# google/ghost-dataplane

Measured on AMD Instinct MI355X. Metric: Mpkt/s device-resident coprocessor NF pipeline (64B pkts); HBM GB/s vs peak, higher is better.
Workload: dtype u32

## Files before the change

### ghost-dataplane_amd/csrc/cop_device.h

```cpp
#ifndef COP_DEVICE_H
#define COP_DEVICE_H

#include <hip/hip_runtime.h>
#include <stdint.h>

#include "cop_kernels.h"

namespace copd {

constexpr int BLOCK = COPK_BLOCK;
constexpr int WAVES = BLOCK / 64;

typedef uint32_t u32x2 __attribute__((ext_vector_type(2)));
typedef uint32_t u32x4 __attribute__((ext_vector_type(4)));
typedef uint32_t u32x4a __attribute__((ext_vector_type(4), aligned(4)));
typedef uint32_t u32x2a __attribute__((ext_vector_type(2), aligned(4)));

__device__ __forceinline__ uint32_t bswap32(uint32_t x) { return __builtin_bswap32(x); }

__device__ __forceinline__ void lb_store(unsigned long long *p, unsigned long long v)
{
    __hip_atomic_store(p, v, __ATOMIC_RELAXED, __HIP_MEMORY_SCOPE_AGENT);
}

// ... 66 lines not shown
__device__ __forceinline__ void lds_stage(uint32_t *lds_dst, const void *gsrc, uint32_t n16, int lane, int wave)
{
    const uint4 *g = (const uint4 *)gsrc;
    for (uint32_t c = (uint32_t)wave; c * 64u < n16; c += WAVES) {
        const uint32_t i = c * 64u + (uint32_t)lane;
        if (i < n16)
            __builtin_amdgcn_global_load_lds((const __attribute__((address_space(1))) void *)(g + i),
                                             (__attribute__((address_space(3))) void *)(lds_dst + c * 256u),
                                             16, 0, 0);
    }
}

__device__ __forceinline__ uint32_t ivt_search(const uint32_t *S, uint32_t m, uint32_t ib, uint32_t lv, uint32_t ip)
{
    const uint16_t *idx = (const uint16_t *)(S + m);
    const uint32_t b = ip >> (32u - ib);
    uint32_t k = idx[b];
    const uint32_t hi = idx[b + 1];
    for (uint32_t step = (1u << lv) >> 1; step; step >>= 1) {
        const uint32_t c = min(k + step, hi);
        if (S[c] <= ip) k = c;
    }
    return k;
}

#ifndef COPK_IVT_VALUE
#define COPK_IVT_VALUE 1
#endif
__device__ __forceinline__ uint32_t ivt_value(const uint32_t *S, const uint32_t *V, uint32_t m, uint32_t ib, uint32_t lv,
                                              uint32_t ip)
{
    if (!COPK_IVT_VALUE || lv == 0) return V[ivt_search(S, m, ib, lv, ip)];
    const uint16_t *idx = (const uint16_t *)(S + m);
    const uint32_t b = ip >> (32u - ib);
    uint32_t k = idx[b];
    const uint32_t hi = idx[b + 1];
    for (uint32_t step = (1u << lv) >> 1; step > 1; step >>= 1) {
        const uint32_t c = min(k + step, hi);
        if (S[c] <= ip) k = c;
    }
    const uint32_t c = min(k + 1, hi);
    const uint32_t sc = S[c], vk = V[k], vc = V[c];
    return sc <= ip ? vc : vk;
}

constexpr int LB_GROUPS = 4;
constexpr uint32_t LB_GAVE_UP = 0xFFFFFFFFu;
__device__ __forceinline__ uint32_t look_back(unsigned long long *chain, uint32_t stride, uint32_t j, uint32_t agg,
                                              uint32_t epoch, uint32_t *err, int lane, const uint32_t *exitw = nullptr,
                                              uint32_t spin_log2 = 22)
{
    const unsigned long long ep = (unsigned long long)epoch << 32;
    if (j == 0) {
        if (lane == 0) lb_store(&chain[0], ep | (2ull << 30) | agg);
        return 0;
    }
    if (lane == 0) lb_store(&chain[(size_t)j * stride], ep | (1ull << 30) | agg);
    uint32_t excl = 0;
    int qhi = (int)j - 1;
    uint32_t spins = 0;
    for (;;) {
        unsigned long long v[LB_GROUPS];
#pragma unroll
        for (int r = 0; r < LB_GROUPS; r++) {
            const int idx = qhi - r * 64 - lane;
            v[r] = idx >= 0 ? lb_load(&chain[(size_t)idx * stride]) : 0ull;
        }
        int consumed = 0;
        bool done = false;
#pragma unroll
        for (int r = 0; r < LB_GROUPS; r++) {
            const bool inb = qhi - r * 64 - lane >= 0;
            const uint32_t flag = (uint32_t)(v[r] >> 30) & 3u;
            const bool ok = inb && (uint32_t)(v[r] >> 32) == epoch && flag != 0u;
            const unsigned long long m_incl = __ballot(ok && flag == 2u);
            const unsigned long long m_bad = __ballot(inb && !ok);
            const int first_incl = m_incl ? __ffsll((long long)m_incl) - 1 : 64;
            const int first_bad = m_bad ? __ffsll((long long)m_bad) - 1 : 64;
            const int upto = min(first_incl + 1, first_bad);
            uint32_t val = lane < upto ? ((uint32_t)v[r] & 0x3FFFFFFFu) : 0u;
#pragma unroll
            for (int off = 32; off; off >>= 1) val += __shfl_xor(val, off);
            excl += val;
            consumed += upto;
            if (first_incl < first_bad) {
                done = true;
                break;
            }
            if (upto < 64) break;
        }
        if (done) break;
        qhi -= consumed;
        if (consumed == 0) {
            if (++spins > (1u << spin_log2)) {
                if (lane == 0) *err = 1u;
                if (exitw) return LB_GAVE_UP;
                break;
            }
            if (exitw && (spins & 63u) == 0 &&
                __hip_atomic_load(exitw, __ATOMIC_RELAXED, __HIP_MEMORY_SCOPE_AGENT) == COPK_PMD_ABORT)
                return LB_GAVE_UP;
            __builtin_amdgcn_s_sleep(1);
        }
    }
    if (lane == 0) lb_store(&chain[(size_t)j * stride], ep | (2ull << 30) | (excl + agg));
    return excl;
}

__device__ __forceinline__ uint32_t look_back_seg(unsigned long long *chain, uint32_t K, uint32_t gi, uint32_t agg,
                                                  uint32_t epoch, uint32_t *err, int lane)
{
    const uint32_t seg = K == 1 ? 64u : K == 2 ? 32u : K <= 4 ? 16u : 8u;
    const uint32_t q = (uint32_t)lane / seg, r = (uint32_t)lane % seg;
    const bool active = q < K;
    const unsigned long long segm = seg == 64 ? ~0ull : ((1ull << seg) - 1ull) << (q * seg);
    const uint32_t sh = seg == 64 ? 0u : q * seg;
    const unsigned long long ep = (unsigned long long)epoch << 32;
    uint32_t excl = 0;
    int qhi = (int)gi - 1;
    bool done = !active || gi == 0;
    uint32_t spins = 0;
    while (__ballot(!done)) {
        const int idx = qhi - (int)r;
        const bool inb = !done && idx >= 0;
        const unsigned long long v = inb ? lb_load(&chain[(size_t)idx * K + q]) : 0ull;
        const uint32_t flag = (uint32_t)(v >> 30) & 3u;
        const bool ok = inb && (uint32_t)(v >> 32) == epoch && flag != 0u;
        const unsigned long long mi = (__ballot(ok && flag == 2u) & segm) >> sh;
        const unsigned long long mb = (__ballot(inb && !ok) & segm) >> sh;
        const uint32_t first_incl = mi ? (uint32_t)__ffsll((long long)mi) - 1u : seg;
        const uint32_t first_bad = mb ? (uint32_t)__ffsll((long long)mb) - 1u : seg;
        const uint32_t upto = min(first_incl + 1u, first_bad);
        uint32_t val = (inb && r < upto) ? ((uint32_t)v & 0x3FFFFFFFu) : 0u;
        for (uint32_t off = seg >> 1; off; off >>= 1) val += __shfl_xor(val, (int)off);
        bool stalled = false;
        if (!done) {
            excl += val;
            if (first_incl < first_bad) {
                done = true;
            } else {
                qhi -= (int)upto;
                stalled = upto == 0;
            }
        }
        if (__ballot(stalled)) {
            if (++spins > (1u << 22)) {
                if (lane == 0) *err = 1u;
                break;
            }
            __builtin_amdgcn_s_sleep(1);
        }
    }
    if (active && r == 0 && gi != 0) lb_store(&chain[(size_t)gi * K + q], ep | (2ull << 30) | (excl + agg));
    return excl;
}

__device__ __forceinline__ void lb_publish(unsigned long long *chain, uint32_t K, uint32_t gi, uint32_t agg_q,
                                           uint32_t epoch, int lane)
{
    if ((uint32_t)lane < K)
        lb_store(&chain[(size_t)gi * K + (uint32_t)lane],
                 ((unsigned long long)epoch << 32) | ((gi == 0 ? 2ull : 1ull) << 30) | agg_q);
}

__device__ __forceinline__ uint32_t wave_excl_scan(uint32_t c, int n, int lane, uint32_t *agg)
{
    uint32_t inc = c;
#pragma unroll
    for (int off = 1; off < 64; off <<= 1) {
        const uint32_t u = __shfl_up(inc, off);
        if (lane >= off) inc += u;
    }
    *agg = __shfl(inc, n - 1);
    return inc - c;
}

__device__ __forceinline__ CopKBatch batch_desc(const CopKParams &p, uint32_t b, uint32_t *look_off)
{
    CopKBatch B;
    if (p.ring) {
        const uint32_t slot = (p.rg.first + b) % p.rg.n_slots;
        B.pkts = p.rg.pkts + (size_t)slot * p.rg.pkts_slot_bytes;
        B.offsets = p.rg.offsets ? p.rg.offsets + (size_t)slot * p.rg.offsets_slot_words : nullptr;
        B.results = (uint2 *)p.rg.results + (size_t)slot * p.rg.results_slot;
        B.fwd_idx = p.rg.fwd_idx ? p.rg.fwd_idx + (size_t)slot * p.rg.fwd_slot : nullptr;
        const uint32_t per = p.seg ? (p.rg.n + COPK_SEG - 1u) / COPK_SEG : p.demux ? p.demux : 1u;
        B.fwd_count = p.rg.fwd_count ? p.rg.fwd_count + (size_t)slot * per : nullptr;
        B.n = p.rg.n;
        B.stride = p.rg.stride;
        B.data_off = p.rg.data_off;
        B.ntiles = p.uniform_ntiles;
        *look_off = b * p.uniform_ntiles;
    } else {
        B = p.b[b];
        *look_off = p.look_begin[b];
    }
    return B;
}

__device__ __forceinline__ uint32_t batch_of_tile(const CopKParams &p, uint32_t g)
{
    uint32_t b = 0;
    if (p.uniform_ntiles) {
        b = g / p.uniform_ntiles;
    } else {
#pragma unroll
        for (int q = 1; q < COPK_MAXB; q++) b += (q < (int)p.nb && p.tile_begin[q] <= g) ? 1u : 0u;
    }
    return __builtin_amdgcn_readfirstlane(b);
}

struct StepGeom {
    uint32_t lpk[3], lch[3];
    uint32_t r3;
    int a3, a67, a8;
};

__device__ __forceinline__ StepGeom step_geom(int lane)
{
    StepGeom g;
#pragma unroll
    for (int c = 0; c < 3; c++) {
        const uint32_t q = (uint32_t)(c * 64 + lane);
        g.lpk[c] = q / 3u;
        g.lch[c] = (q % 3u) * 16u;
    }
    g.r3 = (uint32_t)lane % 3u;
    g.a3 = ((3 * lane) & 63) << 2;
    g.a67 = ((3 * lane + 1) & 63) << 2;
    g.a8 = ((3 * lane + 2) & 63) << 2;
    return g;
}

__device__ __forceinline__ __amdgpu_buffer_rsrc_t sys_rsrc(const void *base)
{
    return __builtin_amdgcn_make_buffer_rsrc((void *)base, 0, 0x7FFFFFFF, 0x00020000);
}
__device__ __forceinline__ u32x4 ld_sys16(__amdgpu_buffer_rsrc_t rs, uint32_t off)
{
    return __builtin_amdgcn_raw_buffer_load_b128(rs, (int)off, 0, 1 | 16);
}
__device__ __forceinline__ u32x2 ld_sys8(__amdgpu_buffer_rsrc_t rs, uint32_t off)
{
    return __builtin_amdgcn_raw_buffer_load_b64(rs, (int)off, 0, 1 | 16);
}
__device__ __forceinline__ uint32_t ld_sys4(__amdgpu_buffer_rsrc_t rs, uint32_t off)
{
    return __builtin_amdgcn_raw_buffer_load_b32(rs, (int)off, 0, 1 | 16);
}

__device__ __forceinline__ void load_step(const StepGeom &g, const uint8_t *pk0, uint32_t stride, uint32_t pb,
                                          uint32_t last, u32x4 (&v)[3], bool sys = false)
{
    if (sys) {
        const __amdgpu_buffer_rsrc_t rs = sys_rsrc(pk0);
#pragma unroll
        for (int c = 0; c < 3; c++) v[c] = ld_sys16(rs, min(pb + g.lpk[c], last) * stride + g.lch[c]);
        return;
    }
#pragma unroll
    for (int c = 0; c < 3; c++) {
        const uint32_t ic = min(pb + g.lpk[c], last);
        v[c] = __builtin_nontemporal_load((const u32x4 *)(pk0 + (size_t)ic * stride + g.lch[c]));
    }
}

__device__ __forceinline__ void load_step_imix(const StepGeom &g, const uint8_t *pkts, uint32_t off,
                                               uint32_t data_off, u32x4 (&v)[3], bool sys = false)
{
    uint32_t o[3];
#pragma unroll
    for (int c = 0; c < 3; c++)
        o[c] = (uint32_t)__builtin_amdgcn_ds_bpermute((int)(g.lpk[c] << 2), (int)off) + data_off + g.lch[c];
    if (sys) {
        const __amdgpu_buffer_rsrc_t rs = sys_rsrc(pkts);
#pragma unroll
        for (int c = 0; c < 3; c++) v[c] = ld_sys16(rs, o[c]);
        return;
    }
#pragma unroll
    for (int c = 0; c < 3; c++) v[c] = __builtin_nontemporal_load((const u32x4 *)(pkts + o[c]));
}

__device__ __forceinline__ uint32_t load_off_imix(const uint32_t *offsets, uint32_t pb, int lane, uint32_t last,
                                                  bool sys = false)
{
    const uint32_t ic = min(pb + (uint32_t)lane, last);
    return sys ? ld_sys4(sys_rsrc(offsets), ic * 4u) : offsets[ic];
}

__device__ __forceinline__ void gather_step(const StepGeom &g, const u32x4 (&v)[3], uint32_t &w3, uint32_t &w6,
                                            uint32_t &w7, uint32_t &w8)
{
    const uint32_t c0w = g.r3 == 0 ? v[0].w : g.r3 == 1 ? v[2].w : v[1].w;
    const uint32_t c1z = g.r3 == 0 ? v[1].z : g.r3 == 1 ? v[0].z : v[2].z;
    const uint32_t c1w = g.r3 == 0 ? v[1].w : g.r3 == 1 ? v[0].w : v[2].w;
    const uint32_t c2x = g.r3 == 0 ? v[2].x : g.r3 == 1 ? v[1].x : v[0].x;
    w3 = (uint32_t)__builtin_amdgcn_ds_bpermute(g.a3, (int)c0w);
    w6 = (uint32_t)__builtin_amdgcn_ds_bpermute(g.a67, (int)c1z);
    w7 = (uint32_t)__builtin_amdgcn_ds_bpermute(g.a67, (int)c1w);
    w8 = (uint32_t)__builtin_amdgcn_ds_bpermute(g.a8, (int)c2x);
}

struct Opt {
    uint32_t demux;
    uint32_t port_stats;
    uint32_t dbg;
    unsigned long long *rule_hits;
};

__device__ __forceinline__ Opt opt_all(const CopKParams &p)
{
    return Opt{p.demux, p.port_stats, p.dbg, p.rule_hits};
}

struct Tables {
    uint32_t *rt_top;
    uint16_t *rt_leaf;
    uint32_t *fw_s, *fw_v, *lp_s, *lp_v;
};

__device__ __forceinline__ uint32_t probe_ld(const uint32_t *a, uint32_t nt)
{
    return nt ? __builtin_nontemporal_load(a) : *a;
}

__device__ __forceinline__ void bkt_issue(const uint32_t *bidx, uint32_t ib, uint32_t ip, bool reach, uint32_t &k0,
                                          uint32_t &k1)
{
    if (reach) {
        const u32x2a x = *(const u32x2a *)(bidx + (ip >> (32u - ib)));
        k0 = x.x;
        k1 = x.y;
    } else {
        k0 = k1 = 0;
    }
}

template <int FW, int LPM, int PPT>
__device__ __forceinline__ void pass1(const CopKParams &p, const Tables &t, const uint32_t (&w3)[PPT],
                                      const uint32_t (&w6)[PPT], const uint32_t (&w7)[PPT],
                                      const uint32_t (&w8)[PPT], uint32_t (&verdict)[PPT], uint32_t (&port)[PPT],
                                      uint32_t (&src)[PPT], uint32_t (&dst)[PPT], uint32_t (&fwe)[PPT],
                                      uint32_t (&lpe)[PPT], uint32_t (&lpe2)[PPT], uint32_t (&fwe2)[PPT])
{
    const bool stageP = (p.stages & COPK_STAGE_PARSE) != 0;
#pragma unroll
    for (int k = 0; k < PPT; k++) {
        verdict[k] = COPK_FORWARD;
        port[k] = 0;
        const uint32_t et = ((w3[k] & 0xFFu) << 8) | ((w3[k] >> 8) & 0xFFu);
        dst[k] = bswap32(__builtin_amdgcn_alignbit(w8[k], w7[k], 16));
        src[k] = bswap32(__builtin_amdgcn_alignbit(w7[k], w6[k], 16));
        if (stageP) {
            if (et != 0x0800u) {
                verdict[k] = COPK_DROP_PARSE;
                port[k] = 0xFFFFu;
            } else {
                const uint32_t idx = dst[k] & 0xFFFFu;
                const uint32_t top = t.rt_top[idx >> 8];
                port[k] = (top & 0x80000000u) ? (uint32_t)t.rt_leaf[((top & 0xFFFFu) << 8) | (idx & 0xFFu)]
                                              : (top & 0xFFFFu);
                if (port[k] == 0xFFFFu) verdict[k] = COPK_DROP_PARSE;
                else if (port[k] >= p.n_ports) verdict[k] = COPK_DROP_NO_PORT;
            }
        }
        const bool reach = verdict[k] == COPK_FORWARD;
        if (FW == COPK_TBL_IVT) fwe[k] = ivt_value(t.fw_s, t.fw_v, p.fw_m, p.fw_ib, p.fw_lv, src[k]);
        if (FW == COPK_TBL_DIR) fwe[k] = reach ? probe_ld(&p.fw_tbl24[src[k] >> 8], p.probe_nt) : 0u;
        if (FW == COPK_TBL_BKT) bkt_issue(p.fw_bidx, p.fw_ib, src[k], reach, fwe[k], fwe2[k]);
        if (LPM == COPK_TBL_IVT) lpe[k] = ivt_value(t.lp_s, t.lp_v, p.lpm_m, p.lpm_ib, p.lpm_lv, dst[k]);
        if (LPM == COPK_TBL_DIR) lpe[k] = reach ? probe_ld(&p.lpm_tbl24[dst[k] >> 8], p.probe_nt) : 0u;
        if (LPM == COPK_TBL_TRIE) lpe[k] = t.lp_s[dst[k] >> 20];
        if (LPM == COPK_TBL_BKT) bkt_issue(p.lpm_bidx, p.lpm_ib, dst[k], reach, lpe[k], lpe2[k]);
    }
}

template <int PPT>
__device__ __forceinline__ void trie_walk(const uint32_t *nodes, const uint32_t *leaves, const uint32_t (&ip)[PPT],
                                          uint32_t (&e)[PPT], const bool (&live)[PPT])
{
    bool in[PPT], lf[PPT];
    bool any = false;
#pragma unroll
    for (int k = 0; k < PPT; k++) {
        in[k] = live[k] && (e[k] & 0x80000000u);
        lf[k] = false;
        any |= in[k];
    }
#pragma unroll
    for (int l = 0; l < 4; l++) {
        if (!__ballot(any)) break;
        const uint32_t sh = l == 0 ? 14u : l == 1 ? 8u : l == 2 ? 2u : 0u;
        const uint32_t msk = l == 3 ? 3u : 63u;
        u32x4a a[PPT];
        u32x2a b[PPT];
#pragma unroll
        for (int k = 0; k < PPT; k++) {
            if (in[k]) {
                const uint32_t *nd = nodes + (size_t)(e[k] & 0x7FFFFFFFu) * 6u;
                a[k] = *(const u32x4a *)nd;
                b[k] = *(const u32x2a *)(nd + 4);
            }
        }
        any = false;
#pragma unroll
        for (int k = 0; k < PPT; k++) {
            if (in[k]) {
                const uint32_t c = (ip[k] >> sh) & msk;
                const unsigned long long vec = a[k].x | ((unsigned long long)a[k].y << 32);
                const unsigned long long lv = a[k].z | ((unsigned long long)a[k].w << 32);
                const unsigned long long upto = (2ull << c) - 1ull;
                if ((vec >> c) & 1ull) {
                    e[k] = 0x80000000u | (b[k].x + (uint32_t)__popcll(vec & upto) - 1u);
                    any = true;
                } else {
                    e[k] = b[k].y + (uint32_t)__popcll(lv & upto) - 1u;
                    in[k] = false;
                    lf[k] = true;
                }
            }
        }
    }
#pragma unroll
    for (int k = 0; k < PPT; k++)
        if (lf[k]) e[k] = leaves[e[k]];
}

template <int PPT>
__device__ __forceinline__ void tbl8_step(const uint32_t *tbl8, uint32_t packed, const uint32_t (&ip)[PPT],
                                          uint32_t (&e)[PPT])
{
    bool ext[PPT];
#pragma unroll
    for (int k = 0; k < PPT; k++) ext[k] = (e[k] & 0x03000000u) == 0x03000000u;
    if (!packed) {
#pragma unroll
        for (int k = 0; k < PPT; k++)
            if (ext[k]) e[k] = tbl8[((size_t)(e[k] & 0x00FFFFFFu) << 8) | (ip[k] & 0xFFu)];
        return;
    }
    unsigned long long h[PPT];
#pragma unroll
    for (int k = 0; k < PPT; k++)
        h[k] = ext[k] ? ((const unsigned long long *)(tbl8 + ((size_t)(e[k] & 0x00FFFFFFu) << 4)))[(ip[k] & 0xFFu) >> 5]
                      : 0ull;
#pragma unroll
    for (int k = 0; k < PPT; k++) {
        if (ext[k]) {
            const uint32_t bit = ip[k] & 31u;
            const uint32_t rank = (uint32_t)(h[k] >> 32) + (uint32_t)__popc((uint32_t)h[k] & (0xFFFFFFFFu >> (31u - bit)));
            e[k] = tbl8[((size_t)(e[k] & 0x00FFFFFFu) << 4) + 16u + rank - 1u];
        }
    }
}

struct T8 {
    bool ext;
    unsigned long long h;
};
__device__ __forceinline__ T8 tbl8_issue(const uint32_t *tbl8, uint32_t packed, uint32_t ip, uint32_t e)
{
    T8 t;
    t.ext = (e & 0x03000000u) == 0x03000000u;
    t.h = 0;
    if (t.ext) {
        if (!packed) t.h = tbl8[((size_t)(e & 0x00FFFFFFu) << 8) | (ip & 0xFFu)];
        else t.h = ((const unsigned long long *)(tbl8 + ((size_t)(e & 0x00FFFFFFu) << 4)))[(ip & 0xFFu) >> 5];
    }
    return t;
}
__device__ __forceinline__ uint32_t tbl8_finish(const uint32_t *tbl8, uint32_t packed, uint32_t ip, uint32_t e,
                                                const T8 &t)
{
    if (!t.ext) return e;
    if (!packed) return (uint32_t)t.h;
    const uint32_t bit = ip & 31u;
    const uint32_t rank = (uint32_t)(t.h >> 32) + (uint32_t)__popc((uint32_t)t.h & (0xFFFFFFFFu >> (31u - bit)));
    return tbl8[((size_t)(e & 0x00FFFFFFu) << 4) + 16u + rank - 1u];
}

template <int PPT>
__device__ __forceinline__ void bkt_step(const uint32_t *pairs, const uint32_t (&ip)[PPT], uint32_t (&e)[PPT],
                                         const uint32_t (&k1)[PPT], const bool (&live)[PPT])
{
    u32x4a q[PPT][4];
#pragma unroll
    for (int k = 0; k < PPT; k++)
        if (live[k]) {
            const uint32_t *b = pairs + 2 * (size_t)e[k];
#pragma unroll
            for (int h = 0; h < 4; h++) q[k][h] = *(const u32x4a *)(b + 4 * h);
        }
    bool more[PPT];
    uint32_t nxt[PPT];
    bool any = false;
#pragma unroll
    for (int k = 0; k < PPT; k++) {
        more[k] = false;
        nxt[k] = 0;
        if (!live[k]) continue;
        const uint32_t k0 = e[k], w = k1[k] - k0;
        uint32_t v = q[k][0].y;
#pragma unroll
        for (int t = 1; t < 8; t++) {
            const u32x4a &c = q[k][t >> 1];
            const uint32_t st = (t & 1) ? c.z : c.x, va = (t & 1) ? c.w : c.y;
            if (w >= (uint32_t)t && ip[k] >= st) v = va;
        }
        e[k] = v;
        more[k] = w > 7u && ip[k] >= q[k][3].z;
        nxt[k] = k0 + 8u;
        any |= more[k];
    }
    while (__ballot(any)) {
        u32x4a c[PPT];
#pragma unroll
        for (int k = 0; k < PPT; k++)
            if (more[k]) c[k] = *(const u32x4a *)(pairs + 2 * (size_t)nxt[k]);
        any = false;
#pragma unroll
        for (int k = 0; k < PPT; k++) {
            if (!more[k]) continue;
            const uint32_t j = nxt[k], hi = k1[k];
            if (ip[k] >= c[k].x) e[k] = c[k].y;
            if (j + 1u <= hi && ip[k] >= c[k].z) e[k] = c[k].w;
            more[k] = j + 1u < hi && ip[k] >= c[k].z;
            any |= more[k];
            nxt[k] = j + 2u;
        }
    }
}

struct BkQ {
    u32x4a q[4];
};
__device__ __forceinline__ BkQ bkt_pairs_issue(const uint32_t *pairs, uint32_t k0, bool live)
{
    BkQ b;
    if (live) {
        const uint32_t *a = pairs + 2 * (size_t)k0;
#pragma unroll
        for (int h = 0; h < 4; h++) b.q[h] = *(const u32x4a *)(a + 4 * h);
    } else {
#pragma unroll
        for (int h = 0; h < 4; h++) b.q[h] = u32x4a{0u, 0u, 0u, 0u};
    }
    return b;
}
__device__ __forceinline__ uint32_t bkt_pairs_finish(const uint32_t *pairs, uint32_t ip, uint32_t k0, uint32_t k1,
                                                     bool live, const BkQ &b)
{
    uint32_t e = k0;
    bool more = false;
    uint32_t nxt = 0;
    if (live) {
        const uint32_t w = k1 - k0;
        uint32_t v = b.q[0].y;
#pragma unroll
        for (int t = 1; t < 8; t++) {
            const u32x4a &c = b.q[t >> 1];
            const uint32_t st = (t & 1) ? c.z : c.x, va = (t & 1) ? c.w : c.y;
            if (w >= (uint32_t)t && ip >= st) v = va;
        }
        e = v;
        more = w > 7u && ip >= b.q[3].z;
        nxt = k0 + 8u;
    }
    while (__ballot(more)) {
        u32x4a c{0u, 0u, 0u, 0u};
        if (more) c = *(const u32x4a *)(pairs + 2 * (size_t)nxt);
        if (more) {
            if (ip >= c.x) e = c.y;
            if (nxt + 1u <= k1 && ip >= c.z) e = c.w;
            more = nxt + 1u < k1 && ip >= c.z;
            nxt += 2u;
        }
    }
    return e;
}

template <int FW, int LPM, int PPT, bool LPM_T8 = true>
__device__ __forceinline__ void pass2(const CopKParams &p, const uint32_t (&w3)[PPT], const uint32_t (&src)[PPT],
                                      const uint32_t (&dst)[PPT], const bool (&valid)[PPT], uint32_t (&fwe)[PPT],
                                      uint32_t (&lpe)[PPT], const uint32_t (&lpe2)[PPT], const uint32_t (&fwe2)[PPT],
                                      uint32_t (&verdict)[PPT], uint32_t (&flags)[PPT], uint32_t (&rnh)[PPT],
                                      uint32_t &c_total, uint32_t &c_notv4)
{
    bool reached[PPT];
#pragma unroll
    for (int k = 0; k < PPT; k++) {
        reached[k] = verdict[k] == COPK_FORWARD;
        flags[k] = 0;
        rnh[k] = 0;
    }
    if (FW == COPK_TBL_DIR) tbl8_step<PPT>(p.fw_tbl8, p.fw_tbl8_packed, src, fwe);
    if (FW == COPK_TBL_BKT) bkt_step<PPT>(p.fw_bpairs, src, fwe, fwe2, reached);
    if (LPM == COPK_TBL_DIR && LPM_T8) tbl8_step<PPT>(p.lpm_tbl8, p.lpm_tbl8_packed, dst, lpe);
    if (LPM == COPK_TBL_TRIE) trie_walk<PPT>(p.lpm_tnodes, p.lpm_tleaves, dst, lpe, reached);
    if (LPM == COPK_TBL_BKT && LPM_T8) bkt_step<PPT>(p.lpm_bpairs, dst, lpe, lpe2, reached);
#pragma unroll
    for (int k = 0; k < PPT; k++) {
        if (!reached[k]) continue;
        if (FW != COPK_TBL_OFF) {
            c_total += valid[k];
            if (((w3[k] >> 20) & 0xFu) != 4u) {
// ... 500 lines not shown
```

### ghost-dataplane_amd/csrc/cop_kernels.h

```cpp
#ifndef COP_KERNELS_H
#define COP_KERNELS_H

#include <hip/hip_runtime.h>
#include <stdint.h>

#define COPK_BLOCK 256
#define COPK_MAXB 32
#define COPK_MAX_LAUNCH_BATCHES 1024
#define COPK_COUNTER_SHARDS 256
static_assert(sizeof(void *) == 8, "64-bit only");
#define COPK_LDS_MISC_WORDS 80
#define COPK_LDS_MISC_EXT_WORDS 408
#define COPK_COALESCED_MIN_STRIDE 48
#define COPK_MAX_DEMUX_PORTS 8
#define COPK_PORT_WORDS 16
#define COPK_STAMP_WG 65536

#define COPK_TBL_OFF 0
#define COPK_TBL_IVT 1
#define COPK_TBL_DIR 2
#define COPK_TBL_TRIE 3
#define COPK_TBL_BKT 4
#define COPK_TRIE_L0 4096u

#define COPK_LAY_SLOTS 0
#define COPK_LAY_IMIX 1
#define COPK_LAY_COALESCED 2
#define COPK_LAY_HDR16 3

#define COPK_STAGE_PARSE 0x1u

#define COPK_FORWARD 0u
#define COPK_DROP_FW 1u
#define COPK_DROP_PARSE 2u
#define COPK_DROP_NOT_IPV4 3u
#define COPK_DROP_NO_PORT 4u
#define COPK_FLAG_ROUTE_HIT 0x1u
#define COPK_FLAG_FW_HIT 0x2u

struct CopKBatch {
    const uint8_t *pkts;
    const uint32_t *offsets;
    void *results;
    uint32_t *fwd_idx;
    uint32_t *fwd_count;
    uint32_t n;
    uint32_t stride;
    uint32_t data_off;
    uint32_t ntiles;
};

struct CopKRing {
    const uint8_t *pkts;
    const uint32_t *offsets;
    void *results;
    uint32_t *fwd_idx;
    uint32_t *fwd_count;
    unsigned long long pkts_slot_bytes, offsets_slot_words, results_slot, fwd_slot;
    uint32_t n_slots, first, n, stride, data_off;
};

struct CopKParams {
    CopKBatch b[COPK_MAXB];
    uint32_t tile_begin[COPK_MAXB];
    uint32_t look_begin[COPK_MAXB];
    CopKRing rg;
    uint32_t ring;
    uint32_t nb;
    uint32_t ntiles;
    uint32_t uniform_ntiles;
    uint32_t stages;
    uint32_t n_ports;
    uint32_t compact;
    uint32_t seg;
    uint32_t static_order;
    uint32_t epoch;
    uint32_t dbg;
    const uint32_t *rt_top;
    const uint16_t *rt_leaf;
    uint32_t rt_nleaf;
    uint32_t fw_m, fw_ib, fw_lv, fw_iw;
    const uint32_t *fw_starts, *fw_vals;
    const uint32_t *fw_tbl24, *fw_tbl8;
    uint32_t fw_tbl8_packed;
    uint32_t lpm_m, lpm_ib, lpm_lv, lpm_iw;
    const uint32_t *lpm_starts, *lpm_vals;
    const uint32_t *lpm_tbl24, *lpm_tbl8;
    uint32_t lpm_tbl8_packed;
    uint32_t probe_nt;
    const uint32_t *lpm_tl0;
    const uint32_t *lpm_tnodes;
    const uint32_t *lpm_tleaves;
    const uint32_t *lpm_bidx, *lpm_bpairs;
    const uint32_t *fw_bidx, *fw_bpairs;
    uint32_t lds_fw_off, lds_lpm_off, lds_misc_off;
    uint32_t lds_stage_off;
    uint32_t lds_rec_off;
    uint32_t rec_paired;
    unsigned long long *tickets;
    unsigned long long *zero_tickets;
    uint32_t zero_lines;
    unsigned long long *look;
    unsigned long long *counters;
    unsigned long long *rule_hits;
    unsigned long long *port_ctr;
    uint32_t demux;
    uint32_t port_stats;
    uint32_t *err;
    unsigned long long *stamps;
    uint32_t *hit_region;
    uint32_t *hit_off;
    uint32_t hit_nb;
    uint32_t hit_reg_words;
    uint32_t lds_hit_off;
};
#define COPK_HIT_SHIFT 14
#define COPK_HIT_MAX_BUCKETS 256
#define COPK_SEG 256

#define COPK_PMD_MAX_RINGS 8
struct CopKPmd {
    CopKParams k;
    CopKRing rings[COPK_PMD_MAX_RINGS];
    unsigned long long seq0r[COPK_PMD_MAX_RINGS];
    uint32_t n_rings;
    const uint32_t *h_n;
    unsigned long long *d_act;
    const unsigned long long *h_posted;
    const uint32_t *h_stop;
    unsigned long long *h_done;
    uint32_t *h_state;
    unsigned long long *d_posted;
    unsigned long long *d_gate;
    uint32_t *d_ctl;
    unsigned long long *slot_tiles;
    uint32_t slot_stride;
    unsigned long long *stamps;
    unsigned long long idle_ticks;
    uint32_t n_work;
    uint32_t relay_stride;
    uint32_t stepwise;
    uint32_t sys_acquire;
    uint32_t test_skip;
    uint32_t poll_backoff;
    uint32_t dyn;
    uint32_t tk_lanes;
    unsigned long long *d_ticket;
};
#define COPK_PMD_TK_LANES 8
#define COPK_PMD_RELAYS 8
#define COPK_PMD_GATE_SHIFT 56
#define COPK_PMD_RUNNING 0u
#define COPK_PMD_STOPPED 1u
#define COPK_PMD_IDLE 2u
#define COPK_PMD_ABORT 3u
#define COPK_PMD_PAUSED 4u

#ifdef __cplusplus
extern "C" {
#endif
hipError_t copk_pmd_launch(const CopKPmd *p, int fw_mode, int lpm_mode, int layout, int ppt, int ext,
                           uint32_t lds_bytes, hipStream_t stream);
hipError_t copk_pmd_occupancy(int fw_mode, int lpm_mode, int layout, int ppt, int ext, uint32_t lds_bytes,
                              int *per_cu);
hipError_t copk_launch(const CopKParams *p, int fw_mode, int lpm_mode, int layout, int ppt,
                       uint32_t grid, uint32_t lds_bytes, hipStream_t stream);
hipError_t copk_hit_count(const CopKParams *p, uint32_t n_tiles, uint32_t tile_pkts, hipStream_t stream);
hipError_t copk_snapshot(unsigned long long *src, uint32_t n_words, unsigned long long *dst, int reset,
                         hipStream_t stream);
#ifdef __cplusplus
}
#endif

#endif
```

### ghost-dataplane_amd/csrc/cop_pmd.hip

```cpp
#include <hip/hip_runtime.h>
#include <stdint.h>

#include <type_traits>

#include "cop_device.h"
#include "cop_kernels.h"
#include "cop_tile.h"

namespace {

using namespace copd;

constexpr uint32_t CENSUS_SPINS = 1u << 21;

__device__ __forceinline__ void st_stamp(unsigned long long *p, unsigned long long v)
{
    __hip_atomic_store(p, v, __ATOMIC_RELAXED, __HIP_MEMORY_SCOPE_AGENT);
}

__device__ __forceinline__ uint32_t ld_agent(uint32_t *p)
{
    return __hip_atomic_load(p, __ATOMIC_RELAXED, __HIP_MEMORY_SCOPE_AGENT);
}

constexpr unsigned long long GATE_POSTED = (1ull << COPK_PMD_GATE_SHIFT) - 1ull;
#ifndef COPK_PMD_NOGATE
#define COPK_PMD_NOGATE 0
#endif

__device__ __forceinline__ unsigned long long ld_u64(const unsigned long long *p)
{
    return __hip_atomic_load(p, __ATOMIC_RELAXED, __HIP_MEMORY_SCOPE_AGENT);
}

#ifndef COPK_PMD_GATE_GUESS
#define COPK_PMD_GATE_GUESS 1
#endif
__device__ __forceinline__ bool gate_publish(unsigned long long *gate, unsigned long long h, unsigned long long guess)
{
    unsigned long long g = COPK_PMD_GATE_GUESS ? guess : ld_u64(gate);
    for (;;) {
        if (g >> COPK_PMD_GATE_SHIFT) return false;
        if ((g & GATE_POSTED) >= h) return true;
        const unsigned long long seen = atomicCAS(gate, g, h);
        if (seen == g) return true;
        g = seen;
    }
}

__device__ __forceinline__ void pmd_leave(const CopKPmd &P, uint32_t why)
{
    for (uint32_t r = 0; r < P.n_rings; r++) {
        unsigned long long *gate = P.d_gate + (size_t)r * 16;
        unsigned long long g = ld_u64(gate);
        while (!(g >> COPK_PMD_GATE_SHIFT)) {
            const unsigned long long seen = atomicCAS(gate, g, g | ((unsigned long long)why << COPK_PMD_GATE_SHIFT));
            if (seen == g) break;
            g = seen;
        }
    }
    if (atomicCAS(&P.d_ctl[0], 0u, why) == 0u)
        __hip_atomic_store(&P.h_state[0], why, __ATOMIC_RELAXED, __HIP_MEMORY_SCOPE_SYSTEM);
}

__device__ __attribute__((unused)) unsigned long long wait_posted(const CopKPmd &P, uint32_t r, uint32_t wr,
                                                                  unsigned long long b, bool leader)
{
    unsigned long long *relay = P.d_posted + ((size_t)r * COPK_PMD_RELAYS + wr % COPK_PMD_RELAYS) * 16;
    unsigned long long *relays = P.d_posted + (size_t)r * COPK_PMD_RELAYS * 16;
    unsigned long long *gate = P.d_gate + (size_t)r * 16;
    const unsigned long long *h_posted = P.h_posted + (size_t)r * 8;
    unsigned long long seen = 0, t_seen = __builtin_amdgcn_s_memrealtime();
    for (uint32_t spins = 0;; spins++) {
        const unsigned long long hp = ld_u64(relay);
        const uint32_t ex = ld_agent(&P.d_ctl[0]);
        unsigned long long h = 0;
        uint32_t stop = 0;
        if (leader) {
            h = __hip_atomic_load(h_posted, __ATOMIC_RELAXED, __HIP_MEMORY_SCOPE_SYSTEM);
            stop = __hip_atomic_load(P.h_stop, __ATOMIC_RELAXED, __HIP_MEMORY_SCOPE_SYSTEM);
        }
        if (hp > b) return hp;
        if (ex) {
            if (ex == COPK_PMD_ABORT) return 0;
            unsigned long long g;
            for (uint32_t k = 0; !((g = ld_u64(gate)) >> COPK_PMD_GATE_SHIFT) && k < (1u << 20); k++)
                __builtin_amdgcn_s_sleep(1);
            const unsigned long long lim = g & GATE_POSTED;
            return (g >> COPK_PMD_GATE_SHIFT) && b < lim ? lim : 0ull;
        }
        if (leader) {
            const unsigned long long now = __builtin_amdgcn_s_memrealtime();
            if (h > hp && (COPK_PMD_NOGATE || gate_publish(gate, h, hp))) {
                for (int x = 0; x < COPK_PMD_RELAYS; x++) atomicMax(relays + x * 16, h);
                if (P.stamps && r == 0) {
                    st_stamp(&P.stamps[(size_t)P.n_work * 8 + (h % 64) * 2], h);
                    st_stamp(&P.stamps[(size_t)P.n_work * 8 + (h % 64) * 2 + 1], now);
                }
                if (h > b) return h;
            }
            if (h != seen) {
                seen = h;
                t_seen = now;
                if (P.n_rings > 1) atomicMax(P.d_act, now);
            }
            if (stop) {
                pmd_leave(P, stop == 2u ? COPK_PMD_PAUSED : COPK_PMD_STOPPED);
            } else if ((spins & 15u) == 15u) {
                if (ld_agent(&P.d_ctl[2])) {
                    pmd_leave(P, COPK_PMD_ABORT);
                } else {
                    unsigned long long last = t_seen;
                    if (P.n_rings > 1) last = max(last, ld_u64(P.d_act));
                    if (now - last > P.idle_ticks) pmd_leave(P, COPK_PMD_IDLE);
                }
            }
        } else {
            for (uint32_t k = spins < 16 ? 0u : P.poll_backoff; k; k--) __builtin_amdgcn_s_sleep(4);
        }
        __builtin_amdgcn_s_sleep(2);
    }
}

__device__ __forceinline__ __attribute__((unused)) CopKBatch pmd_batch(const CopKParams &p, const CopKRing &rg, uint32_t slot, uint32_t n,
                                               uint32_t ntiles)
{
    CopKBatch B;
    B.pkts = rg.pkts + (size_t)slot * rg.pkts_slot_bytes;
    B.offsets = rg.offsets ? rg.offsets + (size_t)slot * rg.offsets_slot_words : nullptr;
    B.results = (uint2 *)rg.results + (size_t)slot * rg.results_slot;
    B.fwd_idx = rg.fwd_idx ? rg.fwd_idx + (size_t)slot * rg.fwd_slot : nullptr;
    const uint32_t per = p.seg ? (rg.n + COPK_SEG - 1u) / COPK_SEG : p.demux ? p.demux : 1u;
    B.fwd_count = rg.fwd_count ? rg.fwd_count + (size_t)slot * per : nullptr;
    B.n = n;
    B.stride = rg.stride;
    B.data_off = rg.data_off;
    B.ntiles = ntiles;
    return B;
}

#ifndef COPK_PMD_WT
#define COPK_PMD_WT 1
#endif
#ifndef COPK_PMD_RELEASE
#define COPK_PMD_RELEASE 0
#endif
#ifndef COPK_PMD_WPE4
#define COPK_PMD_WPE4 5
#endif
#ifndef COPK_PMD_WAVES_PER_EU
#define COPK_PMD_WAVES_PER_EU(ppt) ((ppt) == 8 ? 4 : (ppt) == 4 ? COPK_PMD_WPE4 : 6)
#endif
template <int FW, int LPM, int LAY, int PPT, bool EXT>
__global__ __launch_bounds__(BLOCK, COPK_PMD_WAVES_PER_EU(PPT)) void cop_pmd(const CopKPmd P)
{
    const CopKParams &p = P.k;
    const int tid = threadIdx.x;
    const int lane = tid & 63;
    const int wave = tid >> 6;
    const Opt o = EXT ? opt_all(p) : Opt{0u, 0u, 0u, nullptr};
    extern __shared__ __attribute__((aligned(16))) uint32_t lds[];
    const LdsCarve lc = lds_carve<PPT>(p, lds);
    uint32_t *s_door = lc.s_misc + 36;
    stage_tables<FW, LPM>(p, lc.tb, lane, wave);

    if (tid == 0) {
        atomicAdd(&P.d_ctl[1], 1u);
        uint32_t spins = 0;
        while (ld_agent(&P.d_ctl[1]) < P.n_work && ld_agent(&P.d_ctl[0]) == 0) {
            if (++spins > CENSUS_SPINS) {
                pmd_leave(P, COPK_PMD_ABORT);
                break;
            }
            __builtin_amdgcn_s_sleep(2);
        }
        s_door[2] = ld_agent(&P.d_ctl[0]) == COPK_PMD_ABORT ? 1u : 0u;
    }
    __syncthreads();
    if (s_door[2]) return;
    if (blockIdx.x == 0 && tid == 0)
        __hip_atomic_store(&P.h_state[1], P.n_work, __ATOMIC_RELAXED, __HIP_MEMORY_SCOPE_SYSTEM);

    const uint32_t tpb = p.uniform_ntiles;
    const uint32_t n_slots = p.rg.n_slots;
    constexpr uint32_t TILE = BLOCK * PPT;
    const uint32_t R = P.n_rings;
    const uint32_t r = __builtin_amdgcn_readfirstlane(blockIdx.x % R);
    const uint32_t wr = blockIdx.x / R;
    const uint32_t G = (P.n_work - r + R - 1) / R;
    const CopKRing &rg = P.rings[r];
    const uint32_t rs0 = r * n_slots;
    auto serve = [&](auto steps_c) {
        constexpr bool STEPS = decltype(steps_c)::value;
        unsigned long long b = P.seq0r[r] + wr / tpb;
        uint32_t j = wr % tpb;
        uint32_t slot = (uint32_t)(b % n_slots);
        const uint32_t qb = G / tpb, rb = G % tpb;
        unsigned long long posted = 0;
        const bool leader = wr % P.relay_stride == 0;
        unsigned long long *stamp = P.stamps ? P.stamps + (size_t)blockIdx.x * 8 : nullptr;
        auto count_tile = [&](uint32_t sl, unsigned long long bb) {
            const unsigned long long old = atomicAdd(&P.slot_tiles[(size_t)(rs0 + sl) * P.slot_stride], 1ull);
            const bool last_tile = (old + 1) % tpb == 0;
            if (last_tile) __hip_atomic_store(&P.h_done[rs0 + sl], bb + 1, __ATOMIC_RELAXED, __HIP_MEMORY_SCOPE_SYSTEM);
            if (stamp) {
                st_stamp(&stamp[3], __builtin_amdgcn_s_memrealtime());
                st_stamp(&stamp[5], last_tile ? 1ull : 0ull);
            }
        };
        auto advance = [&] {
            j += rb;
            uint32_t db = qb;
            if (j >= tpb) {
                j -= tpb;
                db++;
            }
            b += db;
            slot += db % n_slots;
            if (slot >= n_slots) slot -= n_slots;
        };
        for (;;) {
            if (stamp && tid == 0) st_stamp(&stamp[0], __builtin_amdgcn_s_memrealtime());
            if (b >= posted) {
                if (tid == 0) {
                    const unsigned long long hp = wait_posted(P, r, wr, b, leader);
                    s_door[0] = (uint32_t)hp;
                    s_door[1] = (uint32_t)(hp >> 32);
                    s_door[2] = hp == 0 ? 1u : 0u;
                }
                lds_barrier();
                posted = ((unsigned long long)s_door[1] << 32) | s_door[0];
                const uint32_t leave = s_door[2];
                lds_barrier();
                if (leave) break;
            }
            if (stamp && tid == 0) {
                st_stamp(&stamp[1], __builtin_amdgcn_s_memrealtime());
                st_stamp(&stamp[4], b);
            }
            uint32_t n = rg.n;
            if (P.h_n) {
                if (tid == 0)
                    s_door[3] = __hip_atomic_load(&P.h_n[rs0 + slot], __ATOMIC_RELAXED, __HIP_MEMORY_SCOPE_SYSTEM);
                lds_barrier();
                n = min(s_door[3], rg.n);
                lds_barrier();
            }
            const uint32_t ntiles = (n + TILE - 1) / TILE;
            const bool wrapped = b >= P.seq0r[r] + n_slots;
            const bool sysld = P.sys_acquire == 3u || (P.sys_acquire == 4u && wrapped);
            if (P.sys_acquire == 1u || (P.sys_acquire == 2u && wrapped)) __builtin_amdgcn_fence(__ATOMIC_ACQUIRE, "");
            int tid_i = tid;
            asm volatile("" : "+v"(tid_i));
            const int lane_i = tid_i & 63;
            const int wave_i = __builtin_amdgcn_readfirstlane(tid_i >> 6);
            bool ok = true;
            if constexpr (STEPS) {
                if (j < ntiles) {
                    const CopKBatch bt = pmd_batch(p, rg, slot, n, ntiles);
                    constexpr int WIN = LPM == COPK_TBL_DIR ? COPK_PMD_WIN_DIR : COPK_PMD_WIN;
                    if (sysld) tile_steps<FW, LPM, PPT, COPK_PMD_WT != 0, 1, WIN, LAY>(p, lc, bt, j, tid_i, lane_i, wave_i);
                    else tile_steps<FW, LPM, PPT, COPK_PMD_WT != 0, 0, WIN, LAY>(p, lc, bt, j, tid_i, lane_i, wave_i);
                }
            } else {
                if (P.test_skip && r == 0 && b == 0 && j + 1 == P.test_skip) {
                    ok = false;
                } else if (j < ntiles) {
                    if (EXT && p.hit_region) {
                        for (uint32_t i = (uint32_t)tid_i; i < p.hit_nb; i += BLOCK) lds[p.lds_hit_off + i] = 0u;
                        lds_barrier();
                    }
                    const LookCtx lk{p.look, (uint32_t)(b + 1), &P.d_ctl[2], &P.d_ctl[0], P.test_skip ? 14u : 22u};
                    body_prio<COPK_PMD_WT != 0, 0>();
                    ok = tile_body<FW, LPM, LAY, PPT, EXT, COPK_PMD_WT != 0>(
                        p, o, lc, pmd_batch(p, rg, slot, n, ntiles), (rs0 + slot) * tpb, j, lk, tid_i, lane_i, wave_i,
                        false, (size_t)(rs0 + slot) * tpb + j, sysld);
                    body_prio<COPK_PMD_WT != 0, 3>();
                }
            }
            if (stamp && tid == 0) st_stamp(&stamp[2], __builtin_amdgcn_s_memrealtime());
            asm volatile("s_waitcnt vmcnt(0)" ::: "memory");
            lds_barrier();
            if (tid == 0 && ok) {
                if (COPK_PMD_RELEASE) {
                    __builtin_amdgcn_fence(__ATOMIC_RELEASE, "agent");
                    asm volatile("s_waitcnt vmcnt(0)" ::: "memory");
                }
                count_tile(slot, b);
            }
            advance();
        }
    };
    constexpr bool DYN_OK = (PPT <= 2 || (COPK_PMD_WIN < PPT ? COPK_PMD_WIN : PPT) <= 2) && LAY == COPK_LAY_COALESCED;
    auto serve_dyn = [&](auto steps_c) {
        constexpr bool STEPS = decltype(steps_c)::value && DYN_OK;
        if constexpr (STEPS) {
            constexpr int W = COPK_PMD_WIN < PPT ? COPK_PMD_WIN : PPT;
            const bool det = P.dyn == 2u;
            const uint32_t nx = (!det && P.tk_lanes > 1 && tpb % P.tk_lanes == 0) ? P.tk_lanes : 1u;
            const uint32_t xl = wr % nx;
            const uint32_t per = tpb / nx;
            unsigned long long *ticket = P.d_ticket + ((size_t)r * COPK_PMD_TK_LANES + xl) * 16;
            uint32_t *s_tk = lc.s_misc + 72;
            unsigned long long *stamp = P.stamps ? P.stamps + (size_t)blockIdx.x * 8 : nullptr;
            const bool leader = wr % P.relay_stride == 0;
            unsigned long long posted = 0;
            unsigned long long pend_old = 0, pend_b = 0;
            uint32_t pend_sl = 0;
            bool pend = false;
            auto pend_flush = [&] {
                if (pend && (pend_old + 1) % tpb == 0)
                    __hip_atomic_store(&P.h_done[rs0 + pend_sl], pend_b + 1, __ATOMIC_RELAXED,
                                       __HIP_MEMORY_SCOPE_SYSTEM);
                pend = false;
            };
            auto claim = [&](unsigned long long cur) {
                return det ? cur + G : __hip_atomic_fetch_add(ticket, 1ull, __ATOMIC_RELAXED, __HIP_MEMORY_SCOPE_AGENT);
            };
            auto tk_get = [&] { return ((unsigned long long)s_tk[1] << 32) | s_tk[0]; };
            if (tid == 0) {
                const unsigned long long t0 = det ? (unsigned long long)wr : claim(0);
                s_tk[0] = (uint32_t)t0;
                s_tk[1] = (uint32_t)(t0 >> 32);
            }
            lds_barrier();
            unsigned long long T = tk_get();
            lds_barrier();
            u32x4 va[W][3], vb[W][3];
            bool loaded = false;
            uint32_t n = rg.n, ntiles = (rg.n + TILE - 1) / TILE;
            const unsigned long long seq0 = P.seq0r[r];
            auto one = [&](u32x4 (&cur)[W][3], u32x4 (&nxt)[W][3]) -> bool {
                int tid_i = tid;
                asm volatile("" : "+v"(tid_i));
                const int lane_i = tid_i & 63;
                const int wave_i = __builtin_amdgcn_readfirstlane(tid_i >> 6);
                const unsigned long long b = seq0 + T / per;
                const uint32_t j = (uint32_t)(T % per) * nx + xl;
                const uint32_t slot = (uint32_t)(b % n_slots);
                if (stamp && tid == 0) {
                    st_stamp(&stamp[0], __builtin_amdgcn_s_memrealtime());
                    st_stamp(&stamp[4], b);
                }
                if (!loaded) {
                    if (b >= posted) {
                        if (tid == 0) {
                            pend_flush();
                            const unsigned long long hp = wait_posted(P, r, wr, b, leader);
                            s_door[0] = (uint32_t)hp;
                            s_door[1] = (uint32_t)(hp >> 32);
                            s_door[2] = hp == 0 ? 1u : 0u;
                        }
                        lds_barrier();
                        posted = ((unsigned long long)s_door[1] << 32) | s_door[0];
                        const uint32_t leave = s_door[2];
                        lds_barrier();
                        if (leave) return true;
                    }
                    n = rg.n;
                    if (P.h_n) {
                        if (tid == 0)
                            s_door[3] = __hip_atomic_load(&P.h_n[rs0 + slot], __ATOMIC_RELAXED, __HIP_MEMORY_SCOPE_SYSTEM);
                        lds_barrier();
                        n = min(s_door[3], rg.n);
                        lds_barrier();
                    }
                    ntiles = (n + TILE - 1) / TILE;
                    const bool wrapped = b >= seq0 + n_slots;
                    if (P.sys_acquire == 1u || (P.sys_acquire == 2u && wrapped))
                        __builtin_amdgcn_fence(__ATOMIC_ACQUIRE, "");
                    const bool sysld = P.sys_acquire == 3u || (P.sys_acquire == 4u && wrapped);
                    step_prio<0>();
                    if (j < ntiles)
                        steps_load<PPT, 0, W>(pmd_batch(p, rg, slot, n, ntiles), j, lane_i, wave_i, cur, sysld);
                }
                if (stamp && tid == 0) st_stamp(&stamp[1], __builtin_amdgcn_s_memrealtime());
                if (tid == 0) {
                    const unsigned long long tn = claim(T);
                    s_tk[0] = (uint32_t)tn;
                    s_tk[1] = (uint32_t)(tn >> 32);
                }
                lds_barrier();
                const unsigned long long Tn = tk_get();
                const unsigned long long bn = seq0 + Tn / per;
                const uint32_t jn = (uint32_t)(Tn % per) * nx + xl;
                const uint32_t sn = (uint32_t)(bn % n_slots);
                const bool pf = bn < posted && !P.h_n;
                if (pf) {
                    const bool wrapped = bn >= seq0 + n_slots;
                    if (P.sys_acquire == 1u || (P.sys_acquire == 2u && wrapped))
                        __builtin_amdgcn_fence(__ATOMIC_ACQUIRE, "");
                    const bool sysld = P.sys_acquire == 3u || (P.sys_acquire == 4u && wrapped);
                    if (jn < ntiles)
                        steps_load<PPT, 0, W>(pmd_batch(p, rg, sn, rg.n, ntiles), jn, lane_i, wave_i, nxt, sysld);
                }
                if (j < ntiles) {
                    const bool sys_t = P.sys_acquire == 3u || (P.sys_acquire == 4u && b >= seq0 + n_slots);
                    tile_steps_v<FW, LPM, PPT, COPK_PMD_WT != 0>(p, lc, pmd_batch(p, rg, slot, n, ntiles), j, tid_i,
                                                                  lane_i, wave_i, cur, sys_t);
                }
                if (stamp && tid == 0) st_stamp(&stamp[2], __builtin_amdgcn_s_memrealtime());
                asm volatile("" ::: "memory");
                __builtin_amdgcn_s_waitcnt(0x0F70);
                asm volatile("" ::: "memory");
                lds_barrier();
                if (tid == 0) {
                    pend_flush();
                    pend_old = atomicAdd(&P.slot_tiles[(size_t)(rs0 + slot) * P.slot_stride], 1ull);
                    pend_b = b;
                    pend_sl = slot;
                    pend = true;
                    if (stamp) st_stamp(&stamp[3], __builtin_amdgcn_s_memrealtime());
                }
                T = Tn;
                loaded = pf;
                return false;
            };
            for (;;) {
                if (one(va, vb)) break;
                if (one(vb, va)) break;
            }
        }
    };
    if (steps_ok<FW, LPM, LAY, EXT>() && p.seg && p.compact && p.rec_paired && P.stepwise) {
        if (DYN_OK && P.dyn) serve_dyn(std::integral_constant<bool, steps_ok<FW, LPM, LAY, EXT>()>{});
        else serve(std::integral_constant<bool, steps_ok<FW, LPM, LAY, EXT>()>{});
    } else {
        serve(std::integral_constant<bool, false>{});
    }
}

template <int FW, int LPM, int LAY, int PPT>
hipError_t pmd_one(const CopKPmd *p, int ext, uint32_t lds, hipStream_t s, int *occ)
{
    if (occ) {
        if (ext) return hipOccupancyMaxActiveBlocksPerMultiprocessor(occ, cop_pmd<FW, LPM, LAY, PPT, true>, BLOCK, lds);
        return hipOccupancyMaxActiveBlocksPerMultiprocessor(occ, cop_pmd<FW, LPM, LAY, PPT, false>, BLOCK, lds);
    }
    const dim3 grid(p->n_work);
    if (ext) hipLaunchKernelGGL((cop_pmd<FW, LPM, LAY, PPT, true>), grid, dim3(BLOCK), lds, s, *p);
    else hipLaunchKernelGGL((cop_pmd<FW, LPM, LAY, PPT, false>), grid, dim3(BLOCK), lds, s, *p);
    return hipGetLastError();
}

template <int FW, int LPM, int LAY>
hipError_t pmd_ppt(const CopKPmd *p, int ppt, int ext, uint32_t lds, hipStream_t s, int *occ)
{
    if (ppt == 8) return pmd_one<FW, LPM, LAY, 8>(p, ext, lds, s, occ);
    if (ppt == 4) return pmd_one<FW, LPM, LAY, 4>(p, ext, lds, s, occ);
    return pmd_one<FW, LPM, LAY, 1>(p, ext, lds, s, occ);
}

template <int FW, int LPM>
hipError_t pmd_lay(const CopKPmd *p, int lay, int ppt, int ext, uint32_t lds, hipStream_t s, int *occ)
{
    if (lay == COPK_LAY_IMIX) return pmd_ppt<FW, LPM, COPK_LAY_IMIX>(p, ppt, ext, lds, s, occ);
    if (lay == COPK_LAY_COALESCED) return pmd_ppt<FW, LPM, COPK_LAY_COALESCED>(p, ppt, ext, lds, s, occ);
    if (lay == COPK_LAY_HDR16) return pmd_ppt<FW, LPM, COPK_LAY_HDR16>(p, ppt, ext, lds, s, occ);
    return pmd_ppt<FW, LPM, COPK_LAY_SLOTS>(p, ppt, ext, lds, s, occ);
}

template <int FW>
hipError_t pmd_lpm(const CopKPmd *p, int lpm, int lay, int ppt, int ext, uint32_t lds, hipStream_t s, int *occ)
{
#ifdef COPK_ISA_PROBE
#ifndef COPK_ISA_LPM
#define COPK_ISA_LPM COPK_TBL_OFF
#endif
    return pmd_one<FW, COPK_ISA_LPM, COPK_LAY_COALESCED, COPK_ISA_PROBE>(p, ext, lds, s, occ);
#else
    if constexpr (FW == COPK_TBL_BKT) {
        if (lpm == COPK_TBL_DIR) return pmd_lay<FW, COPK_TBL_DIR>(p, lay, ppt, ext, lds, s, occ);
        if (lpm == COPK_TBL_BKT) return pmd_lay<FW, COPK_TBL_BKT>(p, lay, ppt, ext, lds, s, occ);
        if (lpm == COPK_TBL_OFF) return pmd_lay<FW, COPK_TBL_OFF>(p, lay, ppt, ext, lds, s, occ);
        return hipErrorInvalidValue;
    } else {
        if (lpm == COPK_TBL_IVT) return pmd_lay<FW, COPK_TBL_IVT>(p, lay, ppt, ext, lds, s, occ);
        if (lpm == COPK_TBL_DIR) return pmd_lay<FW, COPK_TBL_DIR>(p, lay, ppt, ext, lds, s, occ);
        if (lpm == COPK_TBL_TRIE) return pmd_lay<FW, COPK_TBL_TRIE>(p, lay, ppt, ext, lds, s, occ);
        if (lpm == COPK_TBL_BKT) return pmd_lay<FW, COPK_TBL_BKT>(p, lay, ppt, ext, lds, s, occ);
        return pmd_lay<FW, COPK_TBL_OFF>(p, lay, ppt, ext, lds, s, occ);
    }
#endif
}

}

#define COPK_PMD_ARGS const CopKPmd *p, int lpm, int lay, int ppt, int ext, uint32_t lds, hipStream_t s, int *occ
extern "C" hipError_t copk_pmd_fw0(COPK_PMD_ARGS);
extern "C" hipError_t copk_pmd_fw1(COPK_PMD_ARGS);
extern "C" hipError_t copk_pmd_fw2(COPK_PMD_ARGS);
extern "C" hipError_t copk_pmd_fw4(COPK_PMD_ARGS);
#if defined(COPK_FW_PART)
#define COPK_CAT2(a, b) a##b
#define COPK_CAT(a, b) COPK_CAT2(a, b)
extern "C" hipError_t COPK_CAT(copk_pmd_fw, COPK_FW_PART)(COPK_PMD_ARGS)
{
    return pmd_lpm<COPK_FW_PART>(p, lpm, lay, ppt, ext, lds, s, occ);
}
#else
static hipError_t pmd_dispatch(const CopKPmd *p, int fw, int lpm, int lay, int ppt, int ext, uint32_t lds,
                               hipStream_t s, int *occ)
{
    if (fw == COPK_TBL_IVT) return copk_pmd_fw1(p, lpm, lay, ppt, ext, lds, s, occ);
    if (fw == COPK_TBL_DIR) return copk_pmd_fw2(p, lpm, lay, ppt, ext, lds, s, occ);
    if (fw == COPK_TBL_BKT) return copk_pmd_fw4(p, lpm, lay, ppt, ext, lds, s, occ);
    return copk_pmd_fw0(p, lpm, lay, ppt, ext, lds, s, occ);
}

extern "C" hipError_t copk_pmd_launch(const CopKPmd *p, int fw_mode, int lpm_mode, int layout, int ppt, int ext,
                                      uint32_t lds_bytes, hipStream_t stream)
{
    return pmd_dispatch(p, fw_mode, lpm_mode, layout, ppt, ext, lds_bytes, stream, nullptr);
}

extern "C" hipError_t copk_pmd_occupancy(int fw_mode, int lpm_mode, int layout, int ppt, int ext, uint32_t lds_bytes,
                                         int *per_cu)
{
    *per_cu = 0;
    return pmd_dispatch(nullptr, fw_mode, lpm_mode, layout, ppt, ext, lds_bytes, nullptr, per_cu);
}
#endif
```

### ghost-dataplane_amd/csrc/cop_runtime.cpp

```cpp
#include <hip/hip_runtime.h>

#include <dlfcn.h>
#include <errno.h>
#include <stdarg.h>
#include <stdio.h>
#include <stdlib.h>
#include <string.h>
#include <time.h>

#include <algorithm>
#include <atomic>
#include <chrono>
#include <condition_variable>
#include <mutex>
#include <thread>
#include <vector>

#include "cop_gpu.h"
#include "cop_internal.h"
#include "cop_kernels.h"
#include <rccl/rccl.h>

namespace {

// ... 1786 lines not shown
    return rc ? rc : rrc;
}

static int coll_reduce_free(cop_ctx *c, cop_counters *total, uint64_t *rule_hits, uint32_t cap, int reset)
{
    if (c->pmd) {
        if (int rc = pmd_hits_sync(c->pmd, pmd_refresh(c->pmd, 0))) return rc;
    }
    const size_t shard_words = SHARD_WORDS;
    const size_t words = RULE_OFF + c->n_rule_ctr;
    if (c->ctr_sum_words < words) {
        if (c->ctr_sum) (void)hipFree(c->ctr_sum);
        c->ctr_sum = nullptr;
        c->ctr_sum_words = 0;
        HIPCHK(c, hipMalloc(&c->ctr_sum, words * 8));
        c->ctr_sum_words = words;
    }
    const unsigned long long *src = c->counters;
    if (reset) {
        if (c->ctr_snap_words < words) {
            if (c->ctr_snap) (void)hipFree(c->ctr_snap);
            c->ctr_snap = nullptr;
            c->ctr_snap_words = 0;
            HIPCHK(c, hipMalloc(&c->ctr_snap, words * 8));
            c->ctr_snap_words = words;
        }
        hipError_t e = copk_snapshot(c->counters, (uint32_t)words, c->ctr_snap, 1, c->stream);
        if (e != hipSuccess) return set_err(c, -EIO, "snapshot: %s", hipGetErrorString(e));
        src = c->ctr_snap;
    }
    ncclResult_t r = g_rccl.all_reduce(src, c->ctr_sum, words, ncclUint64, ncclSum, c->comm, c->stream);
    if (r != ncclSuccess) return set_err(c, -EIO, "ncclAllReduce: %s", g_rccl.error_string(r));
    HIPCHK(c, hipStreamSynchronize(c->stream));
    if (total) {
        std::vector<uint64_t> sh(shard_words);
        HIPCHK(c, hipMemcpy(sh.data(), c->ctr_sum, shard_words * 8, hipMemcpyDeviceToHost));
        uint64_t sum[COP_N_COUNTERS] = {0};
        for (int s = 0; s < COPK_COUNTER_SHARDS; s++)
            for (int k = 0; k < COP_N_COUNTERS; k++) sum[k] += sh[(size_t)s * COP_N_COUNTERS + k];
        memcpy(total, sum, sizeof(cop_counters));
    }
    const uint32_t k = cap < c->n_rule_ctr ? cap : c->n_rule_ctr;
    if (k) HIPCHK(c, hipMemcpy(rule_hits, c->ctr_sum + RULE_OFF, (size_t)k * 8, hipMemcpyDeviceToHost));
    return (int)c->n_rule_ctr;
}

int cop_dev_alloc(cop_ctx *c, size_t bytes, void **dptr)
{
    if (!c || !dptr) return -EINVAL;
    HIPCHK(c, hipSetDevice(c->device));
    HIPCHK(c, hipMalloc(dptr, bytes ? bytes : 16));
    return 0;
}

int cop_dev_alloc_ex(cop_ctx *c, size_t bytes, uint32_t flags, void **dptr)
{
    if (!c || !dptr || (flags != 0 && flags != COP_ALLOC_UNCACHED && flags != COP_ALLOC_FINEGRAINED)) return -EINVAL;
    if (!flags) return cop_dev_alloc(c, bytes, dptr);
    HIPCHK(c, hipSetDevice(c->device));
    HIPCHK(c, hipExtMallocWithFlags(dptr, bytes ? bytes : 16,
                                    flags == COP_ALLOC_UNCACHED ? hipDeviceMallocUncached : hipDeviceMallocFinegrained));
    return 0;
}

int cop_dev_free(cop_ctx *c, void *dptr)
{
    if (!c) return -EINVAL;
    HIPCHK(c, hipSetDevice(c->device));
    HIPCHK(c, hipFree(dptr));
    return 0;
}

int cop_host_alloc_pinned(cop_ctx *c, size_t bytes, void **hptr)
{
    if (!c || !hptr) return -EINVAL;
    HIPCHK(c, hipSetDevice(c->device));
    HIPCHK(c, hipHostMalloc(hptr, bytes ? bytes : 16, hipHostMallocDefault));
    return 0;
}

int cop_host_alloc_mapped(cop_ctx *c, size_t bytes, void **hptr, void **dptr)
{
    if (!c || !hptr || !dptr) return -EINVAL;
    HIPCHK(c, hipSetDevice(c->device));
    HIPCHK(c, hipHostMalloc(hptr, bytes ? bytes : 16, hipHostMallocMapped | hipHostMallocCoherent));
    hipError_t e = hipHostGetDevicePointer(dptr, *hptr, 0);
    if (e != hipSuccess) {
        (void)hipHostFree(*hptr);
        *hptr = nullptr;
        return set_err(c, -EIO, "mapping: %s", hipGetErrorString(e));
    }
    return 0;
}

int cop_host_free_pinned(cop_ctx *c, void *hptr)
{
    if (!c) return -EINVAL;
    HIPCHK(c, hipHostFree(hptr));
    return 0;
}

int cop_memcpy_h2d(cop_ctx *c, void *dst, const void *src, size_t bytes)
{
    if (!c) return -EINVAL;
    if (int rc = sync_lanes(c)) return rc;
    HIPCHK(c, hipSetDevice(c->device));
    HIPCHK(c, hipMemcpyAsync(dst, src, bytes, hipMemcpyHostToDevice, c->stream));
    HIPCHK(c, hipStreamSynchronize(c->stream));
    return 0;
}

int cop_memcpy_d2h(cop_ctx *c, void *dst, const void *src, size_t bytes)
{
    if (!c) return -EINVAL;
    if (int rc = sync_lanes(c)) return rc;
    HIPCHK(c, hipSetDevice(c->device));
    HIPCHK(c, hipMemcpyAsync(dst, src, bytes, hipMemcpyDeviceToHost, c->stream));
    HIPCHK(c, hipStreamSynchronize(c->stream));
    return 0;
}

int cop_memcpy_d2d(cop_ctx *c, void *dst, const void *src, size_t bytes)
{
    if (!c) return -EINVAL;
    if (int rc = sync_lanes(c)) return rc;
    HIPCHK(c, hipSetDevice(c->device));
    HIPCHK(c, hipMemcpyAsync(dst, src, bytes, hipMemcpyDeviceToDevice, c->stream));
    HIPCHK(c, hipStreamSynchronize(c->stream));
    return 0;
}

int cop_memset_d(cop_ctx *c, void *dst, int value, size_t bytes)
{
    if (!c) return -EINVAL;
    if (int rc = sync_lanes(c)) return rc;
    HIPCHK(c, hipSetDevice(c->device));
    HIPCHK(c, hipMemsetAsync(dst, value, bytes, c->stream));
    HIPCHK(c, hipStreamSynchronize(c->stream));
    return 0;
}

int cop_timer_start(cop_ctx *c)
{
    if (!c) return -EINVAL;
    HIPCHK(c, hipEventRecord(c->t0, c->stream));
    for (int l = 1; l < c->n_lanes; l++) HIPCHK(c, hipStreamWaitEvent(c->lane[l].s, c->t0, 0));
    return 0;
}

int cop_timer_stop(cop_ctx *c, double *ms)
{
    if (!c || !ms) return -EINVAL;
    for (int l = 1; l < c->n_lanes; l++) {
        HIPCHK(c, hipEventRecord(c->lane[l].join, c->lane[l].s));
        HIPCHK(c, hipStreamWaitEvent(c->stream, c->lane[l].join, 0));
    }
    HIPCHK(c, hipEventRecord(c->t1, c->stream));
    HIPCHK(c, hipEventSynchronize(c->t1));
    float f = 0;
    HIPCHK(c, hipEventElapsedTime(&f, c->t0, c->t1));
    *ms = f;
    return 0;
}



struct PmdRing {
    std::atomic<uint64_t> posted{0};
    std::atomic<uint64_t> completed{0};
};

struct cop_pmd {
    cop_ctx *c = nullptr;
    hipStream_t s = nullptr;
    CopKPmd P{};
    int fw_mode = 0, lpm_mode = 0, layout = 0, ppt = 0, ext = 0;
    uint32_t lds_bytes = 0;
    uint8_t *ctl = nullptr;
    volatile uint32_t *h_stop = nullptr;
    volatile uint32_t *h_state = nullptr;
    volatile uint64_t *h_done = nullptr;
    volatile uint32_t *h_n = nullptr;
    uint8_t *dev = nullptr;
    size_t dev_bytes = 0;
    uint32_t n_rings = 1, n_slots = 0, tpb = 0, per_cu = 0, ring_n = 0;
    uint32_t acquire = 4;
    bool dyn = false;
    bool pf = false;
    std::atomic<uint32_t> launches{0};
    uint32_t pauses = 0;
    bool was_live = false;
    bool live = false;
    std::mutex mu;
    PmdRing ring[COPK_PMD_MAX_RINGS];
    bool bins = false;
    hipStream_t hs = nullptr;
    uint64_t counted = 0;
    uint64_t count_synced = 0;
    volatile uint64_t *h_posted(uint32_t r) const { return (volatile uint64_t *)(ctl + 64 * (size_t)r); }
};

constexpr size_t PMD_H_STOP = 512, PMD_H_STATE = 516, PMD_H_DONE = 576;
constexpr size_t PMD_ACT_OFF = 64;
constexpr size_t PMD_GATE_OFF = 1024;
constexpr size_t PMD_RELAY_OFF = 2048;
constexpr size_t PMD_TICKET_OFF = PMD_RELAY_OFF + 128 * COPK_PMD_RELAYS * COPK_PMD_MAX_RINGS;
constexpr size_t PMD_CTL_BYTES = PMD_TICKET_OFF + 128 * COPK_PMD_TK_LANES * COPK_PMD_MAX_RINGS;
static_assert(PMD_GATE_OFF + 128 * COPK_PMD_MAX_RINGS <= PMD_RELAY_OFF, "gates overlap relays");
static_assert(64 * COPK_PMD_MAX_RINGS <= PMD_H_STOP, "posted words overlap the stop word");

static uint64_t pmd_scan(const cop_pmd *m, uint32_t r)
{
    uint64_t c = m->ring[r].completed.load(std::memory_order_relaxed);
    const volatile uint64_t *d = m->h_done + (size_t)r * m->n_slots;
    while (d[c % m->n_slots] == c + 1) c++;
    return c;
}

static int pmd_launch(cop_pmd *m)
{
    cop_ctx *c = m->c;
    HIPCHK(c, hipSetDevice(c->device));
    HIPCHK(c, hipMemsetAsync(m->dev, 0, m->dev_bytes, m->s));
    m->h_state[0] = 0;
    m->h_state[1] = 0;
    *m->h_stop = 0;
    for (uint32_t r = 0; r < m->n_rings; r++) m->P.seq0r[r] = pmd_scan(m, r);
    std::atomic_thread_fence(std::memory_order_seq_cst);
    hipError_t e = copk_pmd_launch(&m->P, m->fw_mode, m->lpm_mode, m->layout, m->ppt, m->ext, m->lds_bytes, m->s);
    if (e != hipSuccess) return set_err(c, -EIO, "pmd launch: %s", hipGetErrorString(e));
    m->launches++;
    m->live = true;
    return 0;
}

static int pmd_join(cop_pmd *m, double timeout_s)
{
    if (!m->live) return 0;
    const auto t0 = std::chrono::steady_clock::now();
    for (;;) {
        hipError_t e = hipStreamQuery(m->s);
        if (e == hipSuccess) break;
        if (e != hipErrorNotReady) return set_err(m->c, -EIO, "pmd: %s", hipGetErrorString(e));
        if (std::chrono::duration<double>(std::chrono::steady_clock::now() - t0).count() > timeout_s)
            return set_err(m->c, -ETIMEDOUT, "pmd: kernel did not leave within %.0f s", timeout_s);
        std::this_thread::sleep_for(std::chrono::microseconds(5));
    }
    m->live = false;
    return 0;
}

static uint64_t pmd_refresh(cop_pmd *m, uint32_t r)
{
    PmdRing &g = m->ring[r];
    const uint64_t posted = g.posted.load(std::memory_order_relaxed);
    const uint64_t c0 = g.completed.load(std::memory_order_relaxed);
    uint64_t c = c0;
    const volatile uint64_t *d = m->h_done + (size_t)r * m->n_slots;
    while (c < posted && d[c % m->n_slots] == c + 1) c++;
    uint64_t cur = c0;
    while (c > cur && !g.completed.compare_exchange_weak(cur, c, std::memory_order_relaxed)) {
    }
    return std::max(c, cur);
}

static int pmd_hits_launch(cop_pmd *m)
{
    if (!m->bins) return 0;
    const CopKParams &p = m->P.k;
    const uint64_t completed = m->ring[0].completed.load(std::memory_order_relaxed);
    while (m->counted < completed) {
        const uint32_t s0 = (uint32_t)(m->counted % m->n_slots);
        const uint32_t k = (uint32_t)std::min<uint64_t>(completed - m->counted, m->n_slots - s0);
        CopKParams q = p;
        q.hit_region = p.hit_region + (size_t)s0 * m->tpb * p.hit_reg_words;
        q.hit_off = p.hit_off + (size_t)s0 * m->tpb * (p.hit_nb + 1);
        hipError_t e = copk_hit_count(&q, k * m->tpb, COPK_BLOCK * (uint32_t)m->ppt, m->hs);
        if (e != hipSuccess) return set_err(m->c, -EIO, "pmd hit count: %s", hipGetErrorString(e));
        m->counted += k;
    }
    return 0;
}

static int pmd_hits_sync(cop_pmd *m, uint64_t upto)
{
    if (!m->bins || m->count_synced >= upto) return 0;
    if (int rc = pmd_hits_launch(m)) return rc;
    HIPCHK(m->c, hipStreamSynchronize(m->hs));
    m->count_synced = m->counted;
    return 0;
}

static int pmd_hits_flush(cop_ctx *c)
{
    cop_pmd *m = c->pmd;
    if (!m || !m->bins) return 0;
    if (m->count_synced >= pmd_refresh(m, 0) && m->ring[0].posted.load() == m->count_synced) return 0;
    if (int rc = pmd_pause(c)) return rc;
    int rc = pmd_hits_sync(m, pmd_refresh(m, 0));
    const int rrc = pmd_resume(c);
    return rc ? rc : rrc;
}

static void pmd_size(cop_pmd *m)
{
    m->P.n_work = (uint32_t)m->c->ncu * m->per_cu;
    m->P.relay_stride = 257;
    if (const char *e = getenv("COP_PMD_RELAY_STRIDE")) m->P.relay_stride = std::max(1u, (uint32_t)atoi(e));
    m->P.poll_backoff = 3;
    m->P.stepwise = getenv("COP_PMD_STEPWISE") && !atoi(getenv("COP_PMD_STEPWISE")) ? 0u : 1u;
    m->P.dyn = m->dyn ? 1u : m->pf ? 2u : 0u;
    m->P.tk_lanes = COPK_PMD_TK_LANES;
    if (const char *e = getenv("COP_PMD_TK_LANES")) m->P.tk_lanes = atoi(e) == 1 ? 1u : (uint32_t)COPK_PMD_TK_LANES;
    if (const char *e = getenv("COP_PMD_BACKOFF")) m->P.poll_backoff = std::min(64u, (uint32_t)atoi(e));
    m->P.sys_acquire = m->acquire;
    if (m->acquire == 4u) {
        for (uint32_t q = 0; q < m->n_rings; q++) {
            hipPointerAttribute_t at;
            if (hipPointerGetAttributes(&at, m->P.rings[q].pkts) == hipSuccess && at.type == hipMemoryTypeHost)
                m->P.sys_acquire = 3;
        }
        (void)hipGetLastError();
        for (uint32_t q = 0; q < m->n_rings && m->P.sys_acquire == 4u; q++) {
            const CopKRing &r = m->P.rings[q];
            bool lined = (uintptr_t)r.pkts % 128u == 0 && r.pkts_slot_bytes % 128u == 0;
            if (r.offsets) lined = lined && (uintptr_t)r.offsets % 128u == 0 && (r.offsets_slot_words * 4u) % 128u == 0;
            if (!lined) m->P.sys_acquire = 3;
        }
    }
    if (const char *e = getenv("COP_PMD_ACQUIRE")) m->P.sys_acquire = std::min(4u, (uint32_t)atoi(e));
    m->P.test_skip = getenv("COP_PMD_TEST_SKIP_TILE") ? (uint32_t)atoi(getenv("COP_PMD_TEST_SKIP_TILE")) + 1u : 0u;
}

static int pmd_census(cop_pmd *m)
{
    const auto t0 = std::chrono::steady_clock::now();
    for (;;) {
        if (m->h_state[1] == m->P.n_work) return 0;
        if (m->h_state[0] == COPK_PMD_ABORT) return 1;
        if (m->h_state[0] != COPK_PMD_RUNNING) return set_err(m->c, -EIO, "pmd: left during the census");
        if (std::chrono::duration<double>(std::chrono::steady_clock::now() - t0).count() > 5.0)
            return set_err(m->c, -ETIMEDOUT, "pmd: no census after 5 s");
        std::this_thread::sleep_for(std::chrono::microseconds(5));
    }
}

static int pmd_prewarm(cop_pmd *m)
{
    cop_ctx *c = m->c;
    const char *env = getenv("COP_PMD_PREWARM");
    if (env && !atoi(env)) return 0;
    HIPCHK(c, hipSetDevice(c->device));
    if (m->bins) {
        hipError_t e = copk_hit_count(&m->P.k, 0, COPK_BLOCK * (uint32_t)m->ppt, m->hs);
        if (e != hipSuccess) return set_err(c, -EIO, "pmd prewarm: %s", hipGetErrorString(e));
        HIPCHK(c, hipStreamSynchronize(m->hs));
    }
    if (int rc = tele_scratch(c)) return rc;
    for (hipStream_t s : {c->tele_stream, c->stream}) {
        hipError_t e = copk_snapshot(c->counters, 1, c->tele_dev, 0, s);
        if (e != hipSuccess) return set_err(c, -EIO, "pmd prewarm: %s", hipGetErrorString(e));
        HIPCHK(c, hipStreamSynchronize(s));
    }
    return 0;
}

static int pmd_launch_resident(cop_pmd *m)
{
    for (;;) {
        if (int rc = pmd_launch(m)) return rc;
        const int st = pmd_census(m);
        if (st == 0) return 0;
        if (st < 0) return st;
        if (int rc = pmd_join(m, 10.0)) return rc;
        if (m->per_cu <= 1 || m->c->ncu * (m->per_cu - 1) < m->n_rings)
            return set_err(m->c, -EIO, "pmd: workers never co-resident");
        m->per_cu--;
        pmd_size(m);
    }
}

static int pmd_revive(cop_pmd *m)
{
    if (m->h_state[0] == COPK_PMD_RUNNING) return 0;
    std::lock_guard<std::mutex> lk(m->mu);
    const uint32_t why = m->h_state[0];
    if (why == COPK_PMD_RUNNING) return 0;
    if (why != COPK_PMD_IDLE && why != COPK_PMD_PAUSED)
        return set_err(m->c, -EIO, "pmd kernel left (%s)", why == COPK_PMD_ABORT ?
                       "abort: workers not co-resident, or a look-back timed out" : "stopped");
    if (int rc = pmd_join(m, 10.0)) return rc;
    return pmd_launch_resident(m);
}

static int pmd_pause(cop_ctx *c)
{
    cop_pmd *m = c->pmd;
    if (!m) return 0;
    m->mu.lock();
    m->was_live = m->live && m->h_state[0] == COPK_PMD_RUNNING;
    if (m->was_live) {
        *m->h_stop = 2u;
        std::atomic_thread_fence(std::memory_order_seq_cst);
    }
    const int rc = pmd_join(m, 10.0);
    if (rc) m->mu.unlock();
    else m->pauses += m->was_live ? 1u : 0u;
    return rc;
}

static int pmd_resume(cop_ctx *c)
{
    cop_pmd *m = c->pmd;
    if (!m) return 0;
    int rc = 0;
    if (m->was_live && !m->live && m->h_state[0] == COPK_PMD_PAUSED) rc = pmd_launch_resident(m);
    m->mu.unlock();
    return rc;
}

static bool pmd_same_geometry(const cop_batch_ring *a, const cop_batch_ring *b)
{
    return a->n_slots == b->n_slots && a->n == b->n && a->stride == b->stride && a->data_off == b->data_off &&
           (a->offsets != nullptr) == (b->offsets != nullptr) && (a->fwd_idx != nullptr) == (b->fwd_idx != nullptr) &&
           (a->fwd_count != nullptr) == (b->fwd_count != nullptr) && a->results_slot == b->results_slot &&
           a->fwd_slot == b->fwd_slot;
}

int cop_pmd_start(cop_ctx *c, const cop_batch_ring *r, cop_pmd **out)
{
    return cop_pmd_start_rings(c, r, 1, 0u, out);
}

int cop_pmd_start_rings(cop_ctx *c, const cop_batch_ring *rings, uint32_t n_rings, uint32_t flags, cop_pmd **out)
{
    return cop_pmd_start_rings_stages(c, rings, n_rings, flags, c ? c->cfg.stages : 0u, out);
}

int cop_pmd_start_rings_stages(cop_ctx *c, const cop_batch_ring *rings, uint32_t n_rings, uint32_t flags,
                               uint32_t stages, cop_pmd **out)
{
    if (!c || !rings || !out || n_rings < 1) return -EINVAL;
    *out = nullptr;
    if (n_rings > COPK_PMD_MAX_RINGS) return set_err(c, -EINVAL, "pmd: %u rings > %d", n_rings, COPK_PMD_MAX_RINGS);
    if (flags & ~(COP_PMD_VARIABLE_N | COP_PMD_SYS_ACQUIRE | COP_PMD_STATIC_SLOTS | COP_PMD_DYNAMIC_TILES))
        return set_err(c, -EINVAL, "pmd: unknown flags %#x", flags);
    if ((flags & COP_PMD_SYS_ACQUIRE) && (flags & COP_PMD_STATIC_SLOTS))
        return set_err(c, -EINVAL, "pmd: COP_PMD_SYS_ACQUIRE and COP_PMD_STATIC_SLOTS contradict");
    if (c->pmd) return set_err(c, -EBUSY, "this context already has a poll-mode kernel");
    const cop_batch_ring *r = &rings[0];
    for (uint32_t q = 0; q < n_rings; q++) {
        const cop_batch_ring *x = &rings[q];
        if (x->n_slots == 0 || x->n == 0 || !x->pkts || !x->results) return set_err(c, -EINVAL, "pmd: empty ring");
        if (q && !pmd_same_geometry(r, x))
            return set_err(c, -EINVAL, "pmd: ring %u's geometry differs from ring 0's (n, slots, stride, layout)", q);
    }
    if (r->n > c->cfg.max_batch) return set_err(c, -EINVAL, "pmd: n %u > max_batch", r->n);
    const bool imix = r->offsets != nullptr;
    const bool compact = (r->fwd_idx || r->fwd_count) && !(c->cfg.flags & COP_CFG_NO_COMPACT);
    const uint32_t lists = (compact && (c->cfg.flags & COP_CFG_DEMUX_PORTS)) ? c->cfg.n_ports : 1u;
    const bool seg = compact && (c->cfg.flags & COP_CFG_SEG_LISTS);
    bool wide = true;
    for (uint32_t q = 0; q < n_rings; q++) {
        const cop_batch_ring *x = &rings[q];
        if (((uintptr_t)x->pkts & 15) || (x->pkts_slot_bytes & 15) || (x->data_off & 15) ||
            (!imix && ((x->stride & 15) || (x->stride < 36 && x->stride != COP_HDR16_STRIDE))))
            return set_err(c, -EINVAL, "pmd: packet starts must be 16-byte aligned");
        if (x->results_slot < x->n || (x->fwd_idx && x->fwd_slot < (uint64_t)x->n * lists))
            return set_err(c, -EINVAL, "pmd: slot sizes smaller than n (x ports with demux)");
        if (int rc = check_seg_ring(c, x, seg)) return rc;
        const uint64_t span = imix ? x->pkts_slot_bytes + x->data_off + 64u
                                   : (uint64_t)x->n * x->stride + x->data_off + 64u;
        if (!(flags & COP_PMD_STATIC_SLOTS) && span > 0x7FFFFFFFull)
            return set_err(c, -EINVAL,
                           "pmd: slots span %llu bytes; coherent slot loads reach 2 GiB (COP_PMD_STATIC_SLOTS for "
                           "slots written once)",
                           (unsigned long long)span);
        wide = wide && ((uintptr_t)x->results & 15) == 0 && (x->results_slot & 1) == 0;
    }
    if (int rc = sync_lanes(c)) return rc;

    cop_pmd *m = new (std::nothrow) cop_pmd();
    if (!m) return -ENOMEM;
    m->c = c;
    m->n_rings = n_rings;
    m->ring_n = r->n;
    m->acquire = (flags & COP_PMD_SYS_ACQUIRE) ? 3u : (flags & COP_PMD_STATIC_SLOTS) ? 0u : 4u;
    Plan pl = plan_launch(c, (uint64_t)r->n * r->n_slots, imix, r->stride);
    int ppt = r->n >= 4u * COPK_BLOCK * 4 ? 4 : 1;
    const char *dyn_env = getenv("COP_PMD_DYN");
    m->dyn = seg && (dyn_env ? atoi(dyn_env) != 0 : (flags & COP_PMD_DYNAMIC_TILES) != 0);
    if (m->dyn && dyn_env && atoi(dyn_env) == 1) ppt = 1;
    m->pf = seg && !m->dyn && getenv("COP_PMD_PF") && atoi(getenv("COP_PMD_PF")) != 0;
    if (c->ppt_override) ppt = c->ppt_override;
    pl.ppt = ppt;
    m->ppt = ppt;
    m->layout = pl.layout;
    m->tpb = (r->n + COPK_BLOCK * ppt - 1) / (COPK_BLOCK * ppt);
    m->n_slots = r->n_slots;
    CopKParams &p = m->P.k;
    memset(&p, 0, sizeof(p));
    p.ring = 1;
    for (uint32_t q = 0; q < n_rings; q++) {
        const cop_batch_ring *x = &rings[q];
        CopKRing &g = m->P.rings[q];
        g.pkts = (const uint8_t *)x->pkts;
        g.offsets = x->offsets;
        g.results = x->results;
        g.fwd_idx = compact ? x->fwd_idx : nullptr;
        g.fwd_count = compact ? x->fwd_count : nullptr;
        g.pkts_slot_bytes = x->pkts_slot_bytes;
        g.offsets_slot_words = x->offsets_slot_words;
        g.results_slot = x->results_slot;
        g.fwd_slot = x->fwd_slot;
        g.n_slots = x->n_slots;
        g.first = 0;
        g.n = x->n;
        g.stride = x->stride;
        g.data_off = x->data_off;
    }
    p.rg = m->P.rings[0];
    m->P.n_rings = n_rings;
    p.nb = 1;
    p.ntiles = m->tpb;
    p.uniform_ntiles = m->tpb;
    p.compact = compact ? 1u : 0u;
    p.seg = seg ? 1u : 0u;
    p.stages = stages;
    p.demux = (compact && (c->cfg.flags & COP_CFG_DEMUX_PORTS)) ? c->cfg.n_ports : 0u;
    int rc = 0;
#define PMD_FAIL(code)       \
    do {                     \
        rc = (code);         \
        goto fail;           \
    } while (0)
    {
        const char *rec_env = getenv("COP_PMD_REC");
        wide = wide && !(rec_env && !strcmp(rec_env, "8"));
        const bool stage_rec = wide && rec_env && !strcmp(rec_env, "stage");
        if ((rc = fill_launch(c, p, ppt, &m->fw_mode, &m->lpm_mode, &m->lds_bytes, stage_rec))) goto fail;
        p.rec_paired = wide && !stage_rec ? 1u : 0u;
        p.dbg = 0;
        p.stamps = nullptr;
        const char *stamps_env = getenv("COP_PMD_STAMPS");
        if (stamps_env && atoi(stamps_env) >= 2) {
            if (hipMalloc(&p.stamps, (size_t)c->ncu * 8 * 8 * 8) != hipSuccess)
                PMD_FAIL(set_err(c, -ENOMEM, "pmd: stamps"));
            if (atoi(stamps_env) == 2) p.dbg = 8;
        }
        if (p.rule_hits && c->hit_bins && n_rings == 1) {
            const uint32_t nb = (c->n_rule_ctr + (1u << COPK_HIT_SHIFT) - 1) >> COPK_HIT_SHIFT;
            const uint32_t reg = COPK_BLOCK * (uint32_t)ppt + 4u * nb;
            const uint32_t base = (m->lds_bytes / 4u + 3u) & ~3u;
            const uint32_t words = ((3u * nb + 5u + 3u) & ~3u) + COPK_BLOCK * (uint32_t)ppt + reg;
            if (nb >= 1 && nb <= COPK_HIT_MAX_BUCKETS && (base + words) * 4u <= 160u * 1024u) {
                const size_t tiles = (size_t)m->n_slots * m->tpb;
                if (hipMalloc(&p.hit_region, tiles * reg * 4) != hipSuccess ||
                    hipMalloc(&p.hit_off, tiles * (nb + 1) * 4) != hipSuccess)
                    PMD_FAIL(set_err(c, -ENOMEM, "pmd: hit regions"));
                if (hipStreamCreateWithFlags(&m->hs, hipStreamNonBlocking) != hipSuccess)
                    PMD_FAIL(set_err(c, -EIO, "pmd: hit stream"));
                p.hit_nb = nb;
                p.hit_reg_words = reg;
                p.lds_hit_off = base;
                m->lds_bytes = (base + words) * 4u;
                m->bins = true;
            }
        }
        m->ext = (p.demux || p.port_stats || p.rule_hits || p.dbg) ? 1 : 0;
        int occ = 0;
        hipError_t e = copk_pmd_occupancy(m->fw_mode, m->lpm_mode, m->layout, ppt, m->ext, m->lds_bytes, &occ);
        if (e != hipSuccess || occ < 1) PMD_FAIL(set_err(c, -EIO, "pmd occupancy: %s (%d)", hipGetErrorString(e), occ));
        occ = std::min(occ, 6);
        if (p.dbg) occ = std::min(occ, 4);
        if (m->bins) occ = std::min(occ, 4);
        if (m->dyn) occ = std::min(occ, 5);
        if (const char *env = getenv("COP_PMD_PER_CU")) occ = std::min(occ, std::max(1, atoi(env)));
        m->per_cu = (uint32_t)occ;
        pmd_size(m);
        m->P.idle_ticks = 100000000ull;
        if (const char *env = getenv("COP_PMD_IDLE_MS")) {
            const unsigned long long ms = std::min<unsigned long long>(strtoull(env, nullptr, 0), 86400000ull);
            m->P.idle_ticks = std::max<unsigned long long>(ms, 1ull) * 100000ull;
        }
        const size_t words = (size_t)n_rings * m->n_slots;
        const bool var_n = (flags & COP_PMD_VARIABLE_N) != 0;
        const size_t ctl_bytes = PMD_H_DONE + words * 8 + (var_n ? words * 4 : 0);
        HIPCHK(c, hipSetDevice(c->device));
        if (hipHostMalloc(&m->ctl, ctl_bytes, hipHostMallocMapped | hipHostMallocCoherent) != hipSuccess)
            PMD_FAIL(set_err(c, -ENOMEM, "pmd: host control block"));
        memset(m->ctl, 0, ctl_bytes);
        void *dctl = nullptr;
        if (hipHostGetDevicePointer(&dctl, m->ctl, 0) != hipSuccess) PMD_FAIL(set_err(c, -EIO, "pmd: mapping"));
        m->h_stop = (volatile uint32_t *)(m->ctl + PMD_H_STOP);
        m->h_state = (volatile uint32_t *)(m->ctl + PMD_H_STATE);
        m->h_done = (volatile uint64_t *)(m->ctl + PMD_H_DONE);
        m->P.h_posted = (const unsigned long long *)dctl;
        m->P.h_stop = (const uint32_t *)((uint8_t *)dctl + PMD_H_STOP);
        m->P.h_state = (uint32_t *)((uint8_t *)dctl + PMD_H_STATE);
        m->P.h_done = (unsigned long long *)((uint8_t *)dctl + PMD_H_DONE);
        if (var_n) {
            m->h_n = (volatile uint32_t *)(m->ctl + PMD_H_DONE + words * 8);
            m->P.h_n = (const uint32_t *)((uint8_t *)dctl + PMD_H_DONE + words * 8);
        }
        m->P.slot_stride = 520;
        if (const char *e = getenv("COP_PMD_SLOT_STRIDE")) m->P.slot_stride = std::max(1u, (uint32_t)atoi(e));
        const size_t look_off = (PMD_CTL_BYTES + words * m->P.slot_stride * 8 + 255) & ~(size_t)255;
        const size_t look_words = (compact && !seg) ? words * m->tpb * (p.demux ? p.demux : 1u) : 0;
        m->dev_bytes = look_off + look_words * 8;
        if (getenv("COP_PMD_STAMPS")) {
            if (hipMalloc(&m->P.stamps, ((size_t)m->P.n_work * 8 + 128) * 8) != hipSuccess)
                PMD_FAIL(set_err(c, -ENOMEM, "pmd: stamps"));
            (void)hipMemset(m->P.stamps, 0, ((size_t)m->P.n_work * 8 + 128) * 8);
            (void)hipDeviceSynchronize();
        }
        if (hipMalloc(&m->dev, m->dev_bytes) != hipSuccess) PMD_FAIL(set_err(c, -ENOMEM, "pmd: device words"));
        if (hipStreamCreateWithFlags(&m->s, hipStreamNonBlocking) != hipSuccess)
            PMD_FAIL(set_err(c, -EIO, "pmd: stream"));
        m->P.d_ctl = (uint32_t *)(m->dev + 8);
        m->P.d_act = (unsigned long long *)(m->dev + PMD_ACT_OFF);
        m->P.d_gate = (unsigned long long *)(m->dev + PMD_GATE_OFF);
        m->P.d_posted = (unsigned long long *)(m->dev + PMD_RELAY_OFF);
        m->P.d_ticket = (unsigned long long *)(m->dev + PMD_TICKET_OFF);
        m->P.slot_tiles = (unsigned long long *)(m->dev + PMD_CTL_BYTES);
        p.look = look_words ? (unsigned long long *)(m->dev + look_off) : nullptr;
        p.err = nullptr;
        p.epoch = 0;
        if ((rc = pmd_prewarm(m))) goto fail;
        if ((rc = pmd_launch_resident(m))) {
            (void)pmd_join(m, 10.0);
            goto fail;
        }
    }
#undef PMD_FAIL
    c->pmd = m;
    *out = m;
    return 0;
fail:
    if (m->P.stamps) (void)hipFree(m->P.stamps);
    if (m->P.k.stamps) (void)hipFree(m->P.k.stamps);
    if (m->P.k.hit_region) (void)hipFree(m->P.k.hit_region);
    if (m->P.k.hit_off) (void)hipFree(m->P.k.hit_off);
    if (m->hs) (void)hipStreamDestroy(m->hs);
    if (m->s) (void)hipStreamDestroy(m->s);
    if (m->dev) (void)hipFree(m->dev);
    if (m->ctl) (void)hipHostFree(m->ctl);
    delete m;
    return rc;
}

int cop_pmd_wait_ring(cop_pmd *m, uint32_t ring, uint64_t seq)
{
    if (!m || ring >= m->n_rings) return -EINVAL;
    PmdRing &g = m->ring[ring];
    const uint64_t posted = g.posted.load(std::memory_order_relaxed);
    if (seq > posted)
        return set_err(m->c, -EINVAL, "pmd: ring %u: wait for %llu > %llu posted", ring, (unsigned long long)seq,
                       (unsigned long long)posted);
    const auto t0 = std::chrono::steady_clock::now();
    uint32_t spins = 0;
    for (;;) {
        if (pmd_refresh(m, ring) >= seq) break;
        if (m->h_state[0] != COPK_PMD_RUNNING) {
            if (pmd_refresh(m, ring) >= seq) break;
            if (int rc = pmd_revive(m)) return rc;
        }
        if ((++spins & 1023u) == 0 &&
            std::chrono::duration<double>(std::chrono::steady_clock::now() - t0).count() > 30.0)
            return set_err(m->c, -ETIMEDOUT, "pmd: ring %u: batch %llu not complete after 30 s", ring,
                           (unsigned long long)g.completed.load());
    }
    std::atomic_thread_fence(std::memory_order_seq_cst);
    return 0;
}

int cop_pmd_wait(cop_pmd *m, uint64_t seq) { return cop_pmd_wait_ring(m, 0, seq); }

static int pmd_post(cop_pmd *m, uint32_t r, uint32_t count, uint32_t n_each)
{
    if (count == 0) return 0;
    if (count > m->n_slots) return set_err(m->c, -EINVAL, "pmd: post of %u > %u ring slots", count, m->n_slots);
    PmdRing &g = m->ring[r];
    const uint64_t posted = g.posted.load(std::memory_order_relaxed);
    const uint64_t need = posted + count;
    if (need - g.completed.load(std::memory_order_relaxed) > m->n_slots)
        if (int rc = cop_pmd_wait_ring(m, r, need - m->n_slots)) return rc;
    if (r == 0 && m->bins && need > m->n_slots && m->count_synced < need - m->n_slots) {
        if (int rc = pmd_pause(m->c)) return rc;
        int rc = pmd_hits_sync(m, need - m->n_slots);
        const int rrc = pmd_resume(m->c);
        if (rc || rrc) return rc ? rc : rrc;
    }
    if (int rc = pmd_revive(m)) return rc;
    if (m->h_n)
        for (uint64_t b = posted; b < need; b++)
            m->h_n[(size_t)r * m->n_slots + b % m->n_slots] = n_each ? n_each : m->ring_n;
    std::atomic_thread_fence(std::memory_order_seq_cst);
    *m->h_posted(r) = need;
    g.posted.store(need, std::memory_order_relaxed);
    return 0;
}

int cop_pmd_post_ring(cop_pmd *m, uint32_t ring, uint32_t count)
{
    if (!m || ring >= m->n_rings) return -EINVAL;
    return pmd_post(m, ring, count, 0);
}

int cop_pmd_post(cop_pmd *m, uint32_t count) { return cop_pmd_post_ring(m, 0, count); }

int cop_pmd_post_batch(cop_pmd *m, uint32_t ring, uint32_t n)
{
    if (!m || ring >= m->n_rings) return -EINVAL;
    if (!m->h_n) return set_err(m->c, -EINVAL, "pmd: started without COP_PMD_VARIABLE_N");
    if (n == 0 || n > m->ring_n) return set_err(m->c, -EINVAL, "pmd: batch of %u packets (1..%u)", n, m->ring_n);
    return pmd_post(m, ring, 1, n);
}

uint64_t cop_pmd_posted(const cop_pmd *m) { return m ? m->ring[0].posted.load() : 0; }

uint64_t cop_pmd_posted_ring(const cop_pmd *m, uint32_t ring)
{
    return m && ring < m->n_rings ? m->ring[ring].posted.load() : 0;
}

uint64_t cop_pmd_completed_ring(cop_pmd *m, uint32_t ring)
{
    return m && ring < m->n_rings ? pmd_refresh(m, ring) : 0;
}

int cop_pmd_run(cop_pmd *m, uint64_t count)
{
    if (!m) return -EINVAL;
    const uint32_t chunk = std::max(1u, m->n_slots / 4);
    for (uint64_t done = 0; done < count;) {
        const uint32_t k = (uint32_t)std::min<uint64_t>(chunk, count - done);
        if (int rc = cop_pmd_post(m, k)) return rc;
        done += k;
    }
    return cop_pmd_wait(m, m->ring[0].posted.load());
}

static uint64_t mono_ns()
{
    timespec ts;
    clock_gettime(CLOCK_MONOTONIC, &ts);
    return (uint64_t)ts.tv_sec * 1000000000ull + (uint64_t)ts.tv_nsec;
}

int cop_pmd_run_timed(cop_pmd *m, uint64_t count, uint64_t *t_post_ns, uint64_t *t_done_ns)
{
    if (!m) return -EINVAL;
    const uint64_t t0 = mono_ns();
    const int rc = cop_pmd_run(m, count);
    const uint64_t t1 = mono_ns();
    if (t_post_ns) *t_post_ns = t0;
    if (t_done_ns) *t_done_ns = t1;
    return rc;
}

int cop_pmd_info(const cop_pmd *m, cop_pmd_info_t *out)
{
    if (!m || !out) return -EINVAL;
    out->workers = m->P.n_work;
    out->workers_per_cu = m->per_cu;
    out->tiles_per_batch = m->tpb;
    out->packets_per_tile = COPK_BLOCK * (uint32_t)m->ppt;
    out->launches = m->launches.load();
    out->state = m->h_state[0];
    out->slot_loads = m->P.sys_acquire;
    out->kernel = (uint32_t)m->fw_mode | (uint32_t)m->lpm_mode << 4 | (uint32_t)m->layout << 8 |
                  (uint32_t)(m->ext ? 1 : 0) << 12;
    out->posted = out->completed = 0;
    for (uint32_t r = 0; r < m->n_rings; r++) {
        out->posted += m->ring[r].posted.load();
        out->completed += m->ring[r].completed.load();
    }
    return 0;
}

int cop_pmd_stop(cop_pmd *m)
{
    if (!m) return -EINVAL;
    cop_ctx *c = m->c;
    int rc = 0;
    for (uint32_t r = 0; r < m->n_rings && !rc; r++) rc = cop_pmd_wait_ring(m, r, m->ring[r].posted.load());
    *m->h_stop = 1;
    std::atomic_thread_fence(std::memory_order_seq_cst);
    const int jrc = pmd_join(m, 10.0);
    if (!rc) rc = jrc;
    if (!rc) rc = pmd_hits_sync(m, m->ring[0].completed.load());
    if (m->hs) (void)hipStreamSynchronize(m->hs);
    if (!jrc) {
        if (m->s) (void)hipStreamDestroy(m->s);
        if (m->hs) (void)hipStreamDestroy(m->hs);
        if (m->dev) (void)hipFree(m->dev);
        if (m->ctl) (void)hipHostFree(m->ctl);
        if (m->P.stamps) (void)hipFree(m->P.stamps);
        if (m->P.k.stamps) (void)hipFree(m->P.k.stamps);
        if (m->P.k.hit_region) (void)hipFree(m->P.k.hit_region);
        if (m->P.k.hit_off) (void)hipFree(m->P.k.hit_off);
    }
    if (c->pmd == m) c->pmd = nullptr;
    delete m;
    return rc;
}

int cop_debug_pmd_stamps(cop_pmd *m, uint64_t *out, uint32_t max_words)
{
    if (!m || !m->P.stamps || !out) return -EINVAL;
    const uint32_t n = std::min<uint32_t>(max_words, m->P.n_work * 8 + 128);
    HIPCHK(m->c, hipMemcpy(out, m->P.stamps, (size_t)n * 8, hipMemcpyDeviceToHost));
    const uint32_t n2 = std::min<uint32_t>(max_words - n, m->P.n_work * 8);
    if (n2 && m->P.k.stamps) HIPCHK(m->c, hipMemcpy(out + n, m->P.k.stamps, (size_t)n2 * 8, hipMemcpyDeviceToHost));
    return (int)(n + (m->P.k.stamps ? n2 : 0));
}

int cop_debug_inject(cop_ctx *c, int what, uint32_t count)
{
    if (!c || (what != 1 && what != 2)) return -EINVAL;
    if (what == 1) c->inject_submit = count;
    else c->inject_wait = count;
    return 0;
}

int cop_debug_stamps(cop_ctx *c, uint64_t *out, uint32_t max_words)
{
    if (!c || !c->stamps) return -EINVAL;
    uint32_t n = max_words < COPK_STAMP_WG * 8 ? max_words : COPK_STAMP_WG * 8;
    if (int rc = sync_lanes(c)) return rc;
    HIPCHK(c, hipMemcpy(out, c->stamps, (size_t)n * 8, hipMemcpyDeviceToHost));
    return (int)n;
}

int cop_debug_host_prof(cop_ctx *c, uint64_t *out, uint32_t n, int reset)
{
    if (!c || !out) return -EINVAL;
    for (uint32_t i = 0; i < n && i < 6; i++) out[i] = c->hp[i];
    if (reset) memset(c->hp, 0, sizeof(c->hp));
    return 6;
}

int cop_launch_timing(cop_ctx *c, int enable)
{
    if (!c) return -EINVAL;
    c->timing = enable != 0;
    return 0;
}

int cop_launch_timing_read(cop_ctx *c, double *mean_ms, uint64_t *n, int reset)
{
    if (!c) return -EINVAL;
    for (int l = 0; l < c->n_lanes; l++)
        while (c->lane[l].ev_count) harvest_one(c, c->lane[l]);
    if (mean_ms) *mean_ms = c->ev_n ? c->ev_sum_ms / (double)c->ev_n : 0.0;
    if (n) *n = c->ev_n;
    if (reset) {
        c->ev_sum_ms = 0;
        c->ev_n = 0;
    }
    return 0;
}

}
```

### ghost-dataplane_amd/csrc/cop_tile.h

```cpp
#ifndef COP_TILE_H
#define COP_TILE_H

#include "cop_device.h"

namespace copd {

#ifndef COPK_PHASE_STAMPS
#define COPK_PHASE_STAMPS 0
#endif
#define STAMP(ph)                                                                          \
    do {                                                                                   \
        if (((o.dbg & 8u) || (COPK_PHASE_STAMPS && p.stamps)) && tid == 0) {               \
            __builtin_amdgcn_sched_barrier(0);                                             \
            __hip_atomic_store(&p.stamps[blockIdx.x * 8 + (ph)], __builtin_amdgcn_s_memrealtime(), \
                               __ATOMIC_RELAXED, __HIP_MEMORY_SCOPE_AGENT);                     \
            __builtin_amdgcn_sched_barrier(0);                                             \
        }                                                                                  \
    } while (0)

struct LdsCarve {
    Tables tb;
    CompactLds cl;
    uint32_t *s_tile;
    uint32_t *s_red;
    uint32_t *s_ps;
    uint32_t *s_misc;
};

template <int PPT>
__device__ __forceinline__ LdsCarve lds_carve(const CopKParams &p, uint32_t *lds)
{
    LdsCarve c;
    c.tb.rt_top = lds;
    c.tb.rt_leaf = (uint16_t *)(lds + 256);
    c.tb.fw_s = lds + p.lds_fw_off;
    c.tb.fw_v = c.tb.fw_s + p.fw_m + p.fw_iw;
    c.tb.lp_s = lds + p.lds_lpm_off;
    c.tb.lp_v = c.tb.lp_s + p.lpm_m + p.lpm_iw;
    uint32_t *misc = lds + p.lds_misc_off;
    c.s_misc = misc;
    c.s_tile = misc + 32;
    c.s_red = misc + 40;
    c.cl.cnt = misc;
    c.cl.pref = misc + 33;
    c.cl.dq = misc + COPK_LDS_MISC_WORDS;
    c.cl.dpref = c.cl.dq + COPK_MAX_DEMUX_PORTS * PPT * WAVES;
    c.s_ps = c.cl.dpref + 8;
    c.cl.stage = p.lds_stage_off ? lds + p.lds_stage_off : nullptr;
    return c;
}

template <int FW, int LPM>
__device__ __forceinline__ void stage_tables(const CopKParams &p, const Tables &tb, int lane, int wave)
{
    constexpr bool fw = FW == COPK_TBL_IVT, lpm = LPM == COPK_TBL_IVT, trie = LPM == COPK_TBL_TRIE;
    const StageSeg none{nullptr, nullptr, 0u};
    lds_stage_all(StageSeg{p.rt_top, tb.rt_top, 64u}, StageSeg{p.rt_leaf, (uint32_t *)tb.rt_leaf, p.rt_nleaf * 32u},
                  fw ? StageSeg{p.fw_starts, tb.fw_s, (p.fw_m + p.fw_iw) >> 2} : none,
                  fw ? StageSeg{p.fw_vals, tb.fw_v, p.fw_m >> 2} : none,
                  lpm ? StageSeg{p.lpm_starts, tb.lp_s, (p.lpm_m + p.lpm_iw) >> 2}
                      : trie ? StageSeg{p.lpm_tl0, tb.lp_s, COPK_TRIE_L0 / 4u} : none,
                  lpm ? StageSeg{p.lpm_vals, tb.lp_v, p.lpm_m >> 2} : none, lane, wave);
}

struct HitLds {
    uint32_t *cnt;
    uint32_t *cur;
    uint32_t *wsum;
    uint32_t *off;
    uint32_t *tmp;
    uint32_t *ids;
};

template <int PPT>
__device__ __forceinline__ HitLds hit_lds(const CopKParams &p, uint32_t *lds)
{
    HitLds h;
    const uint32_t nb = p.hit_nb;
    h.cnt = lds + p.lds_hit_off;
    h.cur = h.cnt + nb;
    h.wsum = h.cur + nb;
    h.off = h.wsum + 4;
    h.tmp = h.cnt + ((3u * nb + 5u + 3u) & ~3u);
    h.ids = h.tmp + BLOCK * PPT;
    return h;
}

template <int PPT>
__device__ __forceinline__ void hit_hist(const HitLds &h, const bool (&valid)[PPT], const uint32_t (&flags)[PPT],
                                         const uint32_t (&fwe)[PPT], int tid, bool one)
{
#pragma unroll
    for (int k = 0; k < PPT; k++) {
        const bool hit = valid[k] && (flags[k] & COPK_FLAG_FW_HIT);
        const uint32_t id = fwe[k] & 0x00FFFFFFu;
        if (hit && !one) atomicAdd(&h.cnt[id >> COPK_HIT_SHIFT], 1u);
        h.tmp[k * BLOCK + tid] = hit ? id : 0xFFFFFFFFu;
    }
}

template <int PPT, bool WT>
__device__ __forceinline__ void hit_sort_out(const CopKParams &p, const HitLds &h, int tid, int lane, int wave,
                                             size_t tile)
{
    const uint32_t nb = p.hit_nb;
    uint32_t total;
    if (nb == 1) {
        uint32_t mine = 0;
#pragma unroll
        for (int k = 0; k < PPT; k++) mine += h.tmp[k * BLOCK + tid] != 0xFFFFFFFFu;
        uint32_t agg;
        const uint32_t ex = wave_excl_scan(mine, 64, lane, &agg);
        if (lane == 0) h.wsum[wave] = agg;
        lds_barrier();
        uint32_t pos = ex, all = 0;
        for (int w = 0; w < WAVES; w++) {
            pos += w < wave ? h.wsum[w] : 0u;
            all += h.wsum[w];
        }
#pragma unroll
        for (int k = 0; k < PPT; k++) {
            const uint32_t id = h.tmp[k * BLOCK + tid];
            if (id != 0xFFFFFFFFu) h.ids[pos++] = id;
        }
        total = (all + 3u) & ~3u;
        if ((uint32_t)tid < total - all) h.ids[all + tid] = 0xFFFFFFFFu;
        if (tid == 0) {
            h.off[0] = 0;
            h.off[1] = total;
        }
        lds_barrier();
    } else {
        const uint32_t c = (uint32_t)tid < nb ? h.cnt[tid] : 0u;
        const uint32_t v = (c + 3u) & ~3u;
        uint32_t agg;
        const uint32_t ex = wave_excl_scan(v, 64, lane, &agg);
        if (lane == 0) h.wsum[wave] = agg;
        lds_barrier();
        uint32_t start = ex;
        for (int w = 0; w < wave; w++) start += h.wsum[w];
        if ((uint32_t)tid < nb) {
            h.off[tid] = start;
            h.cur[tid] = start;
            for (uint32_t i = c; i < v; i++) h.ids[start + i] = 0xFFFFFFFFu;
            if ((uint32_t)tid == nb - 1) h.off[nb] = start + v;
        }
        lds_barrier();
        for (int k = 0; k < PPT; k++) {
            const uint32_t id = h.tmp[k * BLOCK + tid];
            if (id != 0xFFFFFFFFu) h.ids[atomicAdd(&h.cur[id >> COPK_HIT_SHIFT], 1u)] = id;
        }
        lds_barrier();
        total = h.off[nb];
    }
    uint32_t *reg = p.hit_region + tile * p.hit_reg_words;
    for (uint32_t c4 = (uint32_t)tid; c4 < total / 4u; c4 += BLOCK)
        st_u32x4<WT>(*(const u32x4 *)&h.ids[4 * c4], reg, 4 * (long)c4);
    for (uint32_t q = (uint32_t)tid; q <= nb; q += BLOCK) st_u32<WT>(h.off[q], &p.hit_off[tile * (nb + 1) + q]);
}

#ifndef COPK_IMIX_COOP
#define COPK_IMIX_COOP 1
#endif
#ifndef COPK_IMIX_STEPS
#define COPK_IMIX_STEPS 1
#endif
#ifndef COPK_BKT_STEPS
#define COPK_BKT_STEPS 1
#endif

template <int FW, int LPM, int LAY, bool EXT>
constexpr bool steps_ok()
{
    return !EXT && FW != COPK_TBL_DIR && FW != COPK_TBL_BKT &&
           ((LAY == COPK_LAY_COALESCED && LPM != COPK_TBL_TRIE && (LPM != COPK_TBL_BKT || COPK_BKT_STEPS)) ||
            (LAY == COPK_LAY_IMIX && COPK_IMIX_STEPS &&
             (LPM == COPK_TBL_DIR || (LPM == COPK_TBL_BKT && COPK_BKT_STEPS))));
}

#ifndef COPK_XP
#define COPK_XP 0
#endif
#ifndef COPK_PMD_WIN
#define COPK_PMD_WIN 1
#endif
#ifndef COPK_PMD_WIN_DIR
#define COPK_PMD_WIN_DIR COPK_PMD_WIN
#endif
template <int PPT, int WIN>
constexpr int win_of()
{
    return WIN < PPT ? WIN : PPT;
}
#ifndef COPK_PMD_PRIO
#define COPK_PMD_PRIO 1
#endif
template <int K>
__device__ __forceinline__ void step_prio()
{
    if constexpr (COPK_PMD_PRIO) __builtin_amdgcn_s_setprio(K >= 3 ? 0 : 3 - K);
}
#ifndef COPK_PMD_PRIO_BODY
#define COPK_PMD_PRIO_BODY 0
#endif
template <bool WT, int K>
__device__ __forceinline__ void body_prio()
{
    if constexpr (WT && COPK_PMD_PRIO_BODY) step_prio<K>();
}
#ifndef COPK_PMD_STAGE_LIST
#define COPK_PMD_STAGE_LIST 1
#endif
#ifndef COPK_SEG_WAVE
#define COPK_SEG_WAVE 1
#endif
#ifndef COPK_WAVE_COUNTERS
#define COPK_WAVE_COUNTERS 1
#endif
template <int PPT>
__device__ __forceinline__ uint32_t step_off(int k, int wave)
{
    if constexpr (COPK_SEG_WAVE && PPT == WAVES) return (uint32_t)(wave * PPT * 64 + k * 64);
    else return (uint32_t)(k * BLOCK + wave * 64);
}

template <int PPT, int K0, int K1, int SYS = 2, int WIN = COPK_PMD_WIN>
__device__ __forceinline__ void steps_load(const CopKBatch &B, uint32_t j, int lane, int wave,
                                           u32x4 (&v)[win_of<PPT, WIN>()][3], bool sys_rt = false)
{
    const bool sys = SYS == 2 ? sys_rt : SYS == 1;
    static_assert(K1 <= win_of<PPT, WIN>(), "steps beyond the window");
    const StepGeom sg = step_geom(lane);
    const uint32_t base = j * (BLOCK * PPT);
    const uint32_t last = B.n ? B.n - 1 : 0u;
#pragma unroll
    for (int k = K0; k < K1; k++)
        load_step(sg, B.pkts + B.data_off, B.stride, base + step_off<PPT>(k, wave), last, v[k], sys);
}

template <int FW, int LPM, int PPT, bool WT, int SYS = 2, int WIN = COPK_PMD_WIN,
          bool STAGE_LIST = COPK_PMD_STAGE_LIST, int LAY = COPK_LAY_COALESCED>
__device__ __forceinline__ void tile_steps_v(const CopKParams &p, const LdsCarve &lc, const CopKBatch &B, uint32_t j,
                                             int tid, int lane, int wave, u32x4 (&v)[win_of<PPT, WIN>()][3],
                                             bool sys_rt = false)
{
    const bool sys = SYS == 2 ? sys_rt : SYS == 1;
    static_assert(COPK_SEG == BLOCK, "one segment per tile step");
    const Tables &tb = lc.tb;
    constexpr int TILE = BLOCK * PPT;
    const uint32_t base = j * TILE;
    const uint32_t last = B.n ? B.n - 1 : 0u;
    const StepGeom sg = step_geom(lane);
    constexpr int W = win_of<PPT, WIN>();
    Counts tot;
    uint32_t *r = (uint32_t *)B.results;
    const int i2 = lane & 31;
    const bool staged = STAGE_LIST && B.fwd_idx && lc.cl.stage && !(COPK_XP & 4);
    uint32_t all_prev = 0;
    auto flush = [&](int k, uint32_t len) {
        const uint32_t cc = (uint32_t)wave * 16u + (uint32_t)(lane & 15);
        const uint32_t pk = base + (uint32_t)k * BLOCK;
        if (lane < 16 && cc * 4u < len)
            st_list_chunk<WT>(&lc.cl.stage[k * BLOCK + cc * 4u], B.fwd_idx, pk + cc * 4u, B.n);
    };
    uint32_t run = 0;
    auto emit = [&](int k, bool valid0, uint32_t verdict0, uint32_t flags0, uint32_t port0, uint32_t rnh0) {
        const uint32_t pk0 = base + k * BLOCK;
        const uint32_t wb = base + step_off<PPT>(k, wave);
        const bool valid[1] = {valid0};
        const uint32_t verdict[1] = {verdict0}, flags[1] = {flags0};
        const Counts c = wave_counts<FW, 1>(valid, verdict, flags);
        tot.total += c.total;
        tot.notv4 += c.notv4;
        tot.fwd += c.fwd;
        tot.dropfw += c.dropfw;
        tot.parse += c.parse;
        tot.noport += c.noport;
        tot.rhit += c.rhit;
        tot.rx += c.rx;
        const unsigned long long bal = __ballot(valid0 && verdict0 == COPK_FORWARD);
        if (lane == 0) {
            lc.cl.cnt[k * WAVES + wave] = (uint32_t)__popcll(bal);
            if (k == PPT - 1) {
                const uint32_t c8[8] = {tot.total, tot.notv4, tot.fwd, tot.dropfw, tot.parse, tot.noport, tot.rhit,
                                        tot.rx};
#pragma unroll
                for (int q = 0; q < 8; q++) lc.s_red[wave * 8 + q] = c8[q];
            }
        }
        const uint32_t rx = verdict0 | (flags0 << 8) | (port0 << 16);
        const uint32_t a0 = (uint32_t)__shfl((int)rx, 2 * i2), a1 = (uint32_t)__shfl((int)rnh0, 2 * i2);
        const uint32_t a2 = (uint32_t)__shfl((int)rx, 2 * i2 + 1), a3 = (uint32_t)__shfl((int)rnh0, 2 * i2 + 1);
        const uint32_t idx = wb + 2u * (uint32_t)i2;
        if (lane < 32 && !(COPK_XP & 2)) {
            if (idx + 1 < B.n) st_u32x4<WT>(u32x4{a0, a1, a2, a3}, r, 2 * (long)idx);
            else if (idx < B.n) st_u32x2<WT>(u32x2{a0, a1}, (u32x2 *)&r[2 * (size_t)idx]);
        }
        if (COPK_XP & 4) {
            if (k == PPT - 1) {
                lds_barrier();
                counters_add(p, lc.s_red, tid);
            }
            return;
        }
        if constexpr (COPK_SEG_WAVE && PPT == WAVES) {
            const uint32_t sb = base + (uint32_t)wave * COPK_SEG;
            const uint32_t rank = run + __builtin_amdgcn_mbcnt_hi((uint32_t)(bal >> 32),
                                                                  __builtin_amdgcn_mbcnt_lo((uint32_t)bal, 0u));
            if (staged) {
                if ((bal >> lane) & 1ull) lc.cl.stage[wave * COPK_SEG + rank] = wb + (uint32_t)lane;
            } else if (B.fwd_idx && ((bal >> lane) & 1ull)) {
                st_u32<WT>(wb + (uint32_t)lane, &B.fwd_idx[sb + rank]);
            }
            run += (uint32_t)__popcll(bal);
            if (k == PPT - 1) {
                if (staged) {
                    asm volatile("" ::: "memory");
                    if ((uint32_t)lane * 4u < run)
                        st_list_chunk<WT>(&lc.cl.stage[wave * COPK_SEG + lane * 4], B.fwd_idx, sb + (uint32_t)lane * 4u,
                                          B.n);
                }
                if (B.fwd_count && lane == 0 && sb < B.n) st_u32<WT>(run, B.fwd_count + sb / COPK_SEG);
                if (COPK_WAVE_COUNTERS) {
                    counters_add_wave(p, tot, lane, blockIdx.x * WAVES + (uint32_t)wave);
                } else {
                    lds_barrier();
                    counters_add(p, lc.s_red, tid);
                }
            }
            return;
        }
        lds_barrier();
        uint32_t off = 0, all = 0;
#pragma unroll
        for (int w = 0; w < WAVES; w++) {
            const uint32_t cw = lc.cl.cnt[k * WAVES + w];
            off += w < wave ? cw : 0u;
            all += cw;
        }
        const uint32_t rank = off + __builtin_amdgcn_mbcnt_hi((uint32_t)(bal >> 32),
                                                             __builtin_amdgcn_mbcnt_lo((uint32_t)bal, 0u));
        if (staged) {
            if (k > 0) flush(k - 1, all_prev);
            if ((bal >> lane) & 1ull) lc.cl.stage[k * BLOCK + rank] = pk0 + tid;
            all_prev = all;
        } else if (B.fwd_idx && ((bal >> lane) & 1ull)) {
            st_u32<WT>(pk0 + tid, &B.fwd_idx[pk0 + rank]);
        }
        if (B.fwd_count && tid == 0 && pk0 < B.n) st_u32<WT>(all, B.fwd_count + pk0 / COPK_SEG);
        if (k == PPT - 1) counters_add(p, lc.s_red, tid);
    };
    auto prio = [&](int k) {
        if (COPK_PMD_PRIO) {
            if (k == 0) step_prio<0>();
            else if (k == 1) step_prio<1>();
            else if (k == 2) step_prio<2>();
            else if (k == 3) step_prio<3>();
        }
    };
    if constexpr (LAY == COPK_LAY_IMIX) {
        static_assert((LPM == COPK_TBL_DIR || LPM == COPK_TBL_BKT) && FW != COPK_TBL_DIR && FW != COPK_TBL_BKT,
                      "IMIX steps: DIR-24-8 or bucketed route");
        struct St {
            uint32_t w3, src, dst, verdict, port, fwe, lpe, lpe2;
            bool valid;
            T8 t8;
            BkQ bq;
        };
        St a{}, b{}, c{};
        u32x4 h[3];
        uint32_t off = load_off_imix(B.offsets, base + step_off<PPT>(0, wave), lane, last, sys);
        load_step_imix(sg, B.pkts, off, B.data_off, h, sys);
        if (PPT > 1) off = load_off_imix(B.offsets, base + step_off<PPT>(1, wave), lane, last, sys);
#pragma unroll
        for (int k = 0; k < PPT + 2; k++) {
            if (k < PPT) {
                uint32_t w3[1], w6[1], w7[1], w8[1];
                prio(k);
                gather_step(sg, h, w3[0], w6[0], w7[0], w8[0]);
                uint32_t verdict[1], port[1], fwe[1], lpe[1], lpe2[1], fwe2[1], src[1], dst[1];
                pass1<FW, LPM, 1>(p, tb, w3, w6, w7, w8, verdict, port, src, dst, fwe, lpe, lpe2, fwe2);
                a = St{w3[0], src[0], dst[0], verdict[0], port[0], fwe[0], lpe[0], lpe2[0],
                       base + step_off<PPT>(k, wave) + (uint32_t)lane < B.n && B.n != 0, T8{false, 0ull}, BkQ{}};
                if (k + 1 < PPT) {
                    load_step_imix(sg, B.pkts, off, B.data_off, h, sys);
                    if (k + 2 < PPT) off = load_off_imix(B.offsets, base + step_off<PPT>(k + 2, wave), lane, last, sys);
                }
            }
            if (k >= 1 && k <= PPT) {
                if constexpr (LPM == COPK_TBL_BKT) b.bq = bkt_pairs_issue(p.lpm_bpairs, b.lpe, b.verdict == COPK_FORWARD);
                else b.t8 = tbl8_issue(p.lpm_tbl8, p.lpm_tbl8_packed, b.dst, b.lpe);
            }
            if (k >= 2) {
                const uint32_t w3[1] = {c.w3}, src[1] = {c.src}, dst[1] = {c.dst}, lpe2[1] = {0}, fwe2[1] = {0};
                const bool valid[1] = {c.valid};
                uint32_t verdict[1] = {c.verdict}, fwe[1] = {c.fwe}, flags[1], rnh[1], ct = 0, cn = 0;
                uint32_t lpe[1];
                if constexpr (LPM == COPK_TBL_BKT)
                    lpe[0] = bkt_pairs_finish(p.lpm_bpairs, c.dst, c.lpe, c.lpe2, c.verdict == COPK_FORWARD, c.bq);
                else lpe[0] = tbl8_finish(p.lpm_tbl8, p.lpm_tbl8_packed, c.dst, c.lpe, c.t8);
                pass2<FW, LPM, 1, false>(p, w3, src, dst, valid, fwe, lpe, lpe2, fwe2, verdict, flags, rnh, ct, cn);
                emit(k - 2, valid[0], verdict[0], flags[0], c.port, rnh[0]);
            }
            c = b;
            b = a;
        }
    } else if constexpr (LPM != COPK_TBL_DIR && LPM != COPK_TBL_BKT) {
#pragma unroll
        for (int k = 0; k < PPT; k++) {
            uint32_t w3[1], w6[1], w7[1], w8[1];
            prio(k);
            gather_step(sg, v[k % W], w3[0], w6[0], w7[0], w8[0]);
            if (k + W < PPT)
                load_step(sg, B.pkts + B.data_off, B.stride, base + step_off<PPT>(k + W, wave), last, v[k % W], sys);
            const bool valid[1] = {base + step_off<PPT>(k, wave) + (uint32_t)lane < B.n && B.n != 0};
            uint32_t verdict[1], port[1], flags[1], rnh[1], fwe[1], lpe[1], lpe2[1], fwe2[1], src[1], dst[1], ct = 0,
                cn = 0;
            if (COPK_XP & 1) {
                verdict[0] = (w3[0] ^ w6[0] ^ w7[0] ^ w8[0]) & 1u;
                port[0] = w7[0] & 3u;
                flags[0] = 0;
                rnh[0] = w8[0];
            } else {
                pass1<FW, LPM, 1>(p, tb, w3, w6, w7, w8, verdict, port, src, dst, fwe, lpe, lpe2, fwe2);
                pass2<FW, LPM, 1>(p, w3, src, dst, valid, fwe, lpe, lpe2, fwe2, verdict, flags, rnh, ct, cn);
            }
            emit(k, valid[0], verdict[0], flags[0], port[0], rnh[0]);
        }
    } else {
        static_assert(FW != COPK_TBL_DIR && FW != COPK_TBL_BKT, "firewall lookups in LDS only");
        struct St {
            uint32_t w3, src, dst, verdict, port, fwe, lpe, lpe2;
            bool valid;
            T8 t8;
            BkQ bq;
        };
        St a{}, b{}, c{};
#pragma unroll
        for (int k = 0; k < PPT + 2; k++) {
            if (k < PPT) {
                uint32_t w3[1], w6[1], w7[1], w8[1];
                prio(k);
                gather_step(sg, v[k % W], w3[0], w6[0], w7[0], w8[0]);
                if (k + W < PPT)
                    load_step(sg, B.pkts + B.data_off, B.stride, base + step_off<PPT>(k + W, wave), last, v[k % W],
                              sys);
                uint32_t verdict[1], port[1], fwe[1], lpe[1], lpe2[1], fwe2[1], src[1], dst[1];
                pass1<FW, LPM, 1>(p, tb, w3, w6, w7, w8, verdict, port, src, dst, fwe, lpe, lpe2, fwe2);
                a = St{w3[0], src[0], dst[0], verdict[0], port[0], fwe[0], lpe[0], lpe2[0],
                       base + step_off<PPT>(k, wave) + (uint32_t)lane < B.n && B.n != 0, T8{false, 0ull}, BkQ{}};
            }
            if (k >= 1 && k <= PPT) {
                if constexpr (LPM == COPK_TBL_BKT) b.bq = bkt_pairs_issue(p.lpm_bpairs, b.lpe, b.verdict == COPK_FORWARD);
                else b.t8 = tbl8_issue(p.lpm_tbl8, p.lpm_tbl8_packed, b.dst, b.lpe);
            }
            if (k >= 2) {
                const uint32_t w3[1] = {c.w3}, src[1] = {c.src}, dst[1] = {c.dst}, lpe2[1] = {0}, fwe2[1] = {0};
                const bool valid[1] = {c.valid};
                uint32_t verdict[1] = {c.verdict}, fwe[1] = {c.fwe}, flags[1], rnh[1], ct = 0, cn = 0;
                uint32_t lpe[1];
                if constexpr (LPM == COPK_TBL_BKT)
                    lpe[0] = bkt_pairs_finish(p.lpm_bpairs, c.dst, c.lpe, c.lpe2, c.verdict == COPK_FORWARD, c.bq);
                else lpe[0] = tbl8_finish(p.lpm_tbl8, p.lpm_tbl8_packed, c.dst, c.lpe, c.t8);
                pass2<FW, LPM, 1, false>(p, w3, src, dst, valid, fwe, lpe, lpe2, fwe2, verdict, flags, rnh, ct, cn);
                emit(k - 2, valid[0], verdict[0], flags[0], c.port, rnh[0]);
            }
            c = b;
            b = a;
        }
    }
    if (staged && !(COPK_SEG_WAVE && PPT == WAVES)) {
        lds_barrier();
        flush(PPT - 1, all_prev);
    }
    step_prio<3>();
}

template <int FW, int LPM, int PPT, bool WT, int SYS, int WIN = COPK_PMD_WIN, int LAY = COPK_LAY_COALESCED>
__device__ __forceinline__ void tile_steps(const CopKParams &p, const LdsCarve &lc, const CopKBatch &B, uint32_t j,
                                           int tid, int lane, int wave)
{
    u32x4 v[win_of<PPT, WIN>()][3];
    step_prio<0>();
    if constexpr (LAY != COPK_LAY_IMIX) steps_load<PPT, 0, win_of<PPT, WIN>(), SYS, WIN>(B, j, lane, wave, v);
    tile_steps_v<FW, LPM, PPT, WT, SYS, WIN, COPK_PMD_STAGE_LIST, LAY>(p, lc, B, j, tid, lane, wave, v);
}

template <int FW, int LPM, int LAY, int PPT, bool EXT, bool WT>
__device__ __forceinline__ bool tile_body(const CopKParams &p, const Opt &o, const LdsCarve &lc, const CopKBatch &B,
                                          uint32_t look_off, uint32_t j, const LookCtx &lk, int tid, int lane, int wave,
                                          bool sync_tables, size_t hit_tile, bool sys = false)
{
    constexpr bool IMIX = LAY == COPK_LAY_IMIX;
    const Tables &tb = lc.tb;
    constexpr int TILE = BLOCK * PPT;
    const uint32_t base = j * TILE;
    uint32_t w3[PPT], w6[PPT], w7[PPT], w8[PPT];
    bool valid[PPT];
    const uint32_t last = B.n ? B.n - 1 : 0u;
    if (LAY == COPK_LAY_COALESCED && B.n) {
        const StepGeom sg = step_geom(lane);
#if defined(COPK_STREAM_W) && COPK_STREAM_W > 0
        constexpr int W = COPK_STREAM_W < PPT ? COPK_STREAM_W : PPT;
        u32x4 v[W][3];
#pragma unroll
        for (int k = 0; k < W; k++) load_step(sg, B.pkts + B.data_off, B.stride, base + k * BLOCK + wave * 64, last, v[k], sys);
#pragma unroll
        for (int k = 0; k < PPT; k++) {
            gather_step(sg, v[k % W], w3[k], w6[k], w7[k], w8[k]);
            if (k + W < PPT) {
                __builtin_amdgcn_sched_barrier(0);
                load_step(sg, B.pkts + B.data_off, B.stride, base + (k + W) * BLOCK + wave * 64, last, v[k % W], sys);
            }
        }
#else
        u32x4 v[PPT][3];
#pragma unroll
        for (int k = 0; k < PPT; k++)
            load_step(sg, B.pkts + B.data_off, B.stride, base + k * BLOCK + wave * 64, last, v[k], sys);
#pragma unroll
        for (int k = 0; k < PPT; k++) gather_step(sg, v[k], w3[k], w6[k], w7[k], w8[k]);
#endif
    } else if (IMIX && COPK_IMIX_COOP && B.n) {
        const StepGeom sg = step_geom(lane);
        uint32_t off[PPT];
#pragma unroll
        for (int k = 0; k < PPT; k++) off[k] = load_off_imix(B.offsets, base + k * BLOCK + wave * 64, lane, last, sys);
        u32x4 v[PPT][3];
#pragma unroll
        for (int k = 0; k < PPT; k++) load_step_imix(sg, B.pkts, off[k], B.data_off, v[k], sys);
#pragma unroll
        for (int k = 0; k < PPT; k++) gather_step(sg, v[k], w3[k], w6[k], w7[k], w8[k]);
    } else if (LAY == COPK_LAY_HDR16 && B.n && B.stride == 12u) {
#pragma unroll
        for (int k = 0; k < PPT; k++) {
            const uint32_t ic = min(base + k * BLOCK + tid, last);
            const uint32_t *r = (const uint32_t *)(B.pkts + B.data_off + (size_t)ic * 12u);
            const uint32_t a = __builtin_nontemporal_load(r), s_ = __builtin_nontemporal_load(r + 1),
                           d_ = __builtin_nontemporal_load(r + 2);
            w3[k] = a;
            w6[k] = s_ << 16;
            w7[k] = (s_ >> 16) | (d_ << 16);
            w8[k] = d_ >> 16;
        }
    } else if (LAY == COPK_LAY_HDR16 && B.n) {
#pragma unroll
        for (int k = 0; k < PPT; k++) {
            const uint32_t ic = min(base + k * BLOCK + tid, last);
            const u32x4 v = sys ? ld_sys16(sys_rsrc(B.pkts + B.data_off), ic * 16u)
                                : __builtin_nontemporal_load((const u32x4 *)(B.pkts + B.data_off + (size_t)ic * 16u));
            w3[k] = v.x;
            w6[k] = v.y;
            w7[k] = v.z;
            w8[k] = v.w;
        }
    } else if (B.n) {
#pragma unroll
        for (int k = 0; k < PPT; k++) {
            const uint32_t ic = min(base + k * BLOCK + tid, last);
            if (sys) {
                const uint32_t po = (IMIX ? ld_sys4(sys_rsrc(B.offsets), ic * 4u) : ic * B.stride) + B.data_off;
                const __amdgpu_buffer_rsrc_t rs = sys_rsrc(B.pkts);
                const u32x4 a = ld_sys16(rs, po + 12u);
                const u32x2 b = ld_sys8(rs, po + 28u);
                w3[k] = a.x;
                w6[k] = a.w;
                w7[k] = b.x;
                w8[k] = b.y;
                continue;
            }
            const uint8_t *pk;
            if (IMIX) pk = B.pkts + B.offsets[ic] + B.data_off;
            else pk = B.pkts + (size_t)ic * B.stride + B.data_off;
            const u32x4a a = *(const u32x4a *)(pk + 12);
            const u32x2a b = *(const u32x2a *)(pk + 28);
            w3[k] = a.x;
            w6[k] = a.w;
            w7[k] = b.x;
            w8[k] = b.y;
        }
    } else {
#pragma unroll
        for (int k = 0; k < PPT; k++) w3[k] = w6[k] = w7[k] = w8[k] = 0;
    }
#pragma unroll
    for (int k = 0; k < PPT; k++) valid[k] = base + k * BLOCK + tid < B.n;
    if (sync_tables) __syncthreads();
    body_prio<WT, 1>();

    uint32_t verdict[PPT], port[PPT], flags[PPT], rnh[PPT], fwe[PPT], lpe[PPT], lpe2[PPT], fwe2[PPT], src[PPT], dst[PPT];
    pass1<FW, LPM, PPT>(p, tb, w3, w6, w7, w8, verdict, port, src, dst, fwe, lpe, lpe2, fwe2);
    if (o.dbg & 8u) {
        uint32_t x = 0;
#pragma unroll
        for (int k = 0; k < PPT; k++) x ^= verdict[k] ^ src[k];
        asm volatile("" ::"v"(x));
    }
    STAMP(2);

    Counts cn;
    pass2<FW, LPM, PPT>(p, w3, src, dst, valid, fwe, lpe, lpe2, fwe2, verdict, flags, rnh, cn.total, cn.notv4);
    body_prio<WT, 2>();
    const bool bins = EXT && FW != COPK_TBL_OFF && p.hit_region != nullptr;
    if (!EXT && p.seg && p.compact && !(o.dbg & 64u)) {
        STAMP(3);
        const bool paired = p.rec_paired != 0;
        bool fwd[PPT];
        Counts dummy;
        auto records = [&] {
            if (paired) store_records_paired<PPT, WT>(B, base, tid, lane, wave, valid, verdict, flags, port, rnh, fwd, dummy);
            else store_records<PPT, WT>(B, base, tid, valid, verdict, flags, port, rnh, fwd, dummy, nullptr);
        };
        seg_epilogue<FW, PPT, WT>(p, B, base, valid, verdict, flags, lc.cl, lc.s_red, tid, lane, wave, records);
        STAMP(5);
        STAMP(6);
        return true;
    }
    if (bins) hit_hist<PPT>(hit_lds<PPT>(p, lc.s_misc - p.lds_misc_off), valid, flags, fwe, tid, p.hit_nb == 1);
    else rule_hit_atomics<FW, PPT>(o, valid, flags, fwe);
    if (o.dbg & 8u) {
        uint32_t x = 0;
#pragma unroll
        for (int k = 0; k < PPT; k++) x ^= verdict[k] ^ rnh[k];
        asm volatile("" ::"v"(x));
    }
    STAMP(3);
    bool fwd[PPT];
#pragma unroll
    for (int k = 0; k < PPT; k++) fwd[k] = valid[k] && verdict[k] == COPK_FORWARD;
    uint32_t *rec_stage = (WT && p.lds_rec_off) ? lc.s_misc - p.lds_misc_off + p.lds_rec_off : nullptr;
    const bool paired = p.rec_paired != 0;
    auto records = [&] {
        if (paired) store_records_paired<PPT, WT>(B, base, tid, lane, wave, valid, verdict, flags, port, rnh, fwd, cn);
        else store_records<PPT, WT>(B, base, tid, valid, verdict, flags, port, rnh, fwd, cn, rec_stage);
    };
    bool ok = true;
    if (p.compact)
        ok = compact_tile<PPT, WT>(lk, o, B, look_off, j, base, fwd, port, p.seg != 0, lc.cl, tid, lane, wave, records);
    else records();
    if (rec_stage) {
        if (!p.compact) lds_barrier();
        copy_out_records<WT>(B.results, base, B.n > base ? min(B.n - base, (uint32_t)TILE) : 0u, rec_stage, tid);
    }
    STAMP(5);
    if (!ok) return false;

    uint32_t prx[COPK_MAX_DEMUX_PORTS] = {}, ptx[COPK_MAX_DEMUX_PORTS] = {};
    if (o.port_stats) port_counts<PPT>(o.port_stats, valid, fwd, port, prx, ptx);
    flush_counters(p, o, cn, prx, ptx, lc.s_red, lc.s_ps, tid, lane, wave);
    if (bins) hit_sort_out<PPT, WT>(p, hit_lds<PPT>(p, lc.s_misc - p.lds_misc_off), tid, lane, wave, hit_tile);
    STAMP(6);
    return true;
}

}

#endif
```

Before: 67190.

## Specialize full tiles, hoist uniform index math, and replace divisions in PMD loop

```diff
diff --git a/ghost-dataplane_amd/csrc/cop_device.h b/ghost-dataplane_amd/csrc/cop_device.h
--- a/ghost-dataplane_amd/csrc/cop_device.h
+++ b/ghost-dataplane_amd/csrc/cop_device.h
@@ -392,6 +392,61 @@
     w8 = (uint32_t)__builtin_amdgcn_ds_bpermute(g.a8, (int)c2x);
 }
 
+struct StepSel {
+    uint32_t m0, m1;
+};
+
+__device__ __forceinline__ StepSel step_sel(const StepGeom &g)
+{
+    StepSel s{g.r3 == 0 ? 0xFFFFFFFFu : 0u, g.r3 == 1 ? 0xFFFFFFFFu : 0u};
+    asm volatile("" : "+v"(s.m0), "+v"(s.m1));
+    return s;
+}
+
+__device__ __forceinline__ uint32_t sel3(const StepSel &s, uint32_t a, uint32_t b, uint32_t c)
+{
+    const uint32_t bc = (b & s.m1) | (c & ~s.m1);
+    return (a & s.m0) | (bc & ~s.m0);
+}
+
+__device__ __forceinline__ void gather_step_sel(const StepGeom &g, const StepSel &s, const u32x4 (&v)[3], uint32_t &w3,
+                                                uint32_t &w6, uint32_t &w7, uint32_t &w8)
+{
+    const uint32_t c0w = sel3(s, v[0].w, v[2].w, v[1].w);
+    const uint32_t c1z = sel3(s, v[1].z, v[0].z, v[2].z);
+    const uint32_t c1w = sel3(s, v[1].w, v[0].w, v[2].w);
+    const uint32_t c2x = sel3(s, v[2].x, v[1].x, v[0].x);
+    w3 = (uint32_t)__builtin_amdgcn_ds_bpermute(g.a3, (int)c0w);
+    w6 = (uint32_t)__builtin_amdgcn_ds_bpermute(g.a67, (int)c1z);
+    w7 = (uint32_t)__builtin_amdgcn_ds_bpermute(g.a67, (int)c1w);
+    w8 = (uint32_t)__builtin_amdgcn_ds_bpermute(g.a8, (int)c2x);
+}
+
+struct StepOff {
+    uint32_t o[3];
+};
+
+__device__ __forceinline__ StepOff step_voff(const StepGeom &g, uint32_t stride)
+{
+    StepOff f;
+#pragma unroll
+    for (int c = 0; c < 3; c++) f.o[c] = g.lpk[c] * stride + g.lch[c];
+    return f;
+}
+
+__device__ __forceinline__ void load_step_full(const uint8_t *ps, const StepOff &f, u32x4 (&v)[3])
+{
+#pragma unroll
+    for (int c = 0; c < 3; c++) v[c] = __builtin_nontemporal_load((const u32x4 *)(ps + f.o[c]));
+}
+
+__device__ __forceinline__ void load_step_full_sys(__amdgpu_buffer_rsrc_t rs, uint32_t soff, const StepOff &f,
+                                                   u32x4 (&v)[3])
+{
+#pragma unroll
+    for (int c = 0; c < 3; c++) v[c] = __builtin_amdgcn_raw_buffer_load_b128(rs, (int)f.o[c], (int)soff, 1 | 16);
+}
+
 struct Opt {
     uint32_t demux;
     uint32_t port_stats;
diff --git a/ghost-dataplane_amd/csrc/cop_kernels.h b/ghost-dataplane_amd/csrc/cop_kernels.h
--- a/ghost-dataplane_amd/csrc/cop_kernels.h
+++ b/ghost-dataplane_amd/csrc/cop_kernels.h
@@ -118,6 +118,30 @@
 #define COPK_HIT_MAX_BUCKETS 256
 #define COPK_SEG 256
 
+struct CopKDiv {
+    uint32_t d, mul, sh1, sh2;
+};
+static inline CopKDiv copk_div_make(uint32_t d)
+{
+    CopKDiv f;
+    uint32_t l = 0;
+    while (l < 32 && (1ull << l) < d) l++;
+    f.d = d;
+    f.mul = (uint32_t)((((1ull << l) - d) << 32) / d + 1ull);
+    f.sh1 = l < 1 ? l : 1u;
+    f.sh2 = l ? l - 1u : 0u;
+    return f;
+}
+__host__ __device__ static inline uint32_t copk_div(uint32_t n, const CopKDiv &f)
+{
+#ifdef __HIP_DEVICE_COMPILE__
+    const uint32_t t = __umulhi(n, f.mul);
+#else
+    const uint32_t t = (uint32_t)(((unsigned long long)n * f.mul) >> 32);
+#endif
+    return (t + ((n - t) >> f.sh1)) >> f.sh2;
+}
+
 #define COPK_PMD_MAX_RINGS 8
 struct CopKPmd {
     CopKParams k;
@@ -146,7 +170,13 @@
     uint32_t dyn;
     uint32_t tk_lanes;
     unsigned long long *d_ticket;
-};
+    uint32_t tk_nx;
+    CopKDiv div_per, div_slots;
+};
+static inline uint32_t copk_pmd_tk_nx(uint32_t dyn, uint32_t tk_lanes, uint32_t tpb)
+{
+    return (dyn == 1u && tk_lanes > 1u && tpb % tk_lanes == 0u) ? tk_lanes : 1u;
+}
 #define COPK_PMD_TK_LANES 8
 #define COPK_PMD_RELAYS 8
 #define COPK_PMD_GATE_SHIFT 56
@@ -161,8 +191,8 @@
 #endif
 hipError_t copk_pmd_launch(const CopKPmd *p, int fw_mode, int lpm_mode, int layout, int ppt, int ext,
                            uint32_t lds_bytes, hipStream_t stream);
-hipError_t copk_pmd_occupancy(int fw_mode, int lpm_mode, int layout, int ppt, int ext, uint32_t lds_bytes,
-                              int *per_cu);
+hipError_t copk_pmd_occupancy(const CopKPmd *p, int fw_mode, int lpm_mode, int layout, int ppt, int ext,
+                              uint32_t lds_bytes, int *per_cu);
 hipError_t copk_launch(const CopKParams *p, int fw_mode, int lpm_mode, int layout, int ppt,
                        uint32_t grid, uint32_t lds_bytes, hipStream_t stream);
 hipError_t copk_hit_count(const CopKParams *p, uint32_t n_tiles, uint32_t tile_pkts, hipStream_t stream);
diff --git a/ghost-dataplane_amd/csrc/cop_pmd.hip b/ghost-dataplane_amd/csrc/cop_pmd.hip
--- a/ghost-dataplane_amd/csrc/cop_pmd.hip
+++ b/ghost-dataplane_amd/csrc/cop_pmd.hip
@@ -22,6 +22,19 @@
 {
     return __hip_atomic_load(p, __ATOMIC_RELAXED, __HIP_MEMORY_SCOPE_AGENT);
 }
+
+#ifndef COPK_PMD_UNI
+#define COPK_PMD_UNI 1
+#endif
+__device__ __forceinline__ __attribute__((unused)) uint32_t uni(uint32_t x) { return COPK_PMD_UNI ? __builtin_amdgcn_readfirstlane(x) : x; }
+__device__ __forceinline__ __attribute__((unused)) unsigned long long uni64(unsigned long long x)
+{
+    return ((unsigned long long)uni((uint32_t)(x >> 32)) << 32) | uni((uint32_t)x);
+}
+#ifndef COPK_PMD_PARK
+#define COPK_PMD_PARK 1
+#endif
+__device__ __forceinline__ __attribute__((unused)) uint32_t lds_uni(const uint32_t *p) { return uni(*p); }
 
 constexpr unsigned long long GATE_POSTED = (1ull << COPK_PMD_GATE_SHIFT) - 1ull;
 #ifndef COPK_PMD_NOGATE
@@ -151,9 +164,29 @@
 #ifndef COPK_PMD_WAVES_PER_EU
 #define COPK_PMD_WAVES_PER_EU(ppt) ((ppt) == 8 ? 4 : (ppt) == 4 ? COPK_PMD_WPE4 : 6)
 #endif
-template <int FW, int LPM, int LAY, int PPT, bool EXT>
+constexpr int LOOP_BODY = 0;
+constexpr int LOOP_STEPS = 1;
+constexpr int LOOP_DYN = 2;
+
+template <int LAY, int PPT>
+constexpr bool dyn_ok()
+{
+    return (PPT <= 2 || (COPK_PMD_WIN < PPT ? COPK_PMD_WIN : PPT) <= 2) && LAY == COPK_LAY_COALESCED;
+}
+
+template <int FW, int LPM, int LAY, int PPT>
+int pmd_loop_of(const CopKPmd *p, int ext)
+{
+    if (!(steps_ok<FW, LPM, LAY, false>() && !ext && p->k.seg && p->k.compact && p->k.rec_paired && p->stepwise))
+        return LOOP_BODY;
+    return dyn_ok<LAY, PPT>() && p->dyn ? LOOP_DYN : LOOP_STEPS;
+}
+
+template <int FW, int LPM, int LAY, int PPT, bool EXT, int LOOP>
 __global__ __launch_bounds__(BLOCK, COPK_PMD_WAVES_PER_EU(PPT)) void cop_pmd(const CopKPmd P)
 {
+    static_assert(LOOP == LOOP_BODY || steps_ok<FW, LPM, LAY, EXT>(), "no step path for this pipeline");
+    static_assert(LOOP != LOOP_DYN || dyn_ok<LAY, PPT>(), "no dynamic tiles for this pipeline");
     const CopKParams &p = P.k;
     const int tid = threadIdx.x;
     const int lane = tid & 63;
@@ -186,22 +219,30 @@
     constexpr uint32_t TILE = BLOCK * PPT;
     const uint32_t R = P.n_rings;
     const uint32_t r = __builtin_amdgcn_readfirstlane(blockIdx.x % R);
-    const uint32_t wr = blockIdx.x / R;
-    const uint32_t G = (P.n_work - r + R - 1) / R;
+    const uint32_t wr = uni(blockIdx.x / R);
+    const uint32_t G = uni((P.n_work - r + R - 1) / R);
     const CopKRing &rg = P.rings[r];
     const uint32_t rs0 = r * n_slots;
     auto serve = [&](auto steps_c) {
         constexpr bool STEPS = decltype(steps_c)::value;
-        unsigned long long b = P.seq0r[r] + wr / tpb;
-        uint32_t j = wr % tpb;
-        uint32_t slot = (uint32_t)(b % n_slots);
-        const uint32_t qb = G / tpb, rb = G % tpb;
+        const unsigned long long seq0 = P.seq0r[r];
+        const uint32_t x0 = uni(wr / tpb);
+        unsigned long long b = seq0 + x0;
+        uint32_t j = wr - x0 * tpb;
+        uint32_t slot0 = uni((uint32_t)(seq0 % n_slots));
+        unsigned long long lap = uni(x0 / n_slots);
+        uint32_t xs = x0 - (uint32_t)lap * n_slots;
+        uint32_t slot = slot0 + xs >= n_slots ? slot0 + xs - n_slots : slot0 + xs;
+        uint32_t qb = uni(G / tpb), rb = G - qb * tpb;
+        uint32_t dl0 = uni(qb / n_slots), ds0 = qb - dl0 * n_slots;
+        uint32_t dl1 = uni((qb + 1) / n_slots), ds1 = qb + 1 - dl1 * n_slots;
         unsigned long long posted = 0;
-        const bool leader = wr % P.relay_stride == 0;
+        const bool leader = uni(wr % P.relay_stride) == 0;
         unsigned long long *stamp = P.stamps ? P.stamps + (size_t)blockIdx.x * 8 : nullptr;
         auto count_tile = [&](uint32_t sl, unsigned long long bb) {
+            const unsigned long long before_last = (lap + 1) * tpb - 1;
             const unsigned long long old = atomicAdd(&P.slot_tiles[(size_t)(rs0 + sl) * P.slot_stride], 1ull);
-            const bool last_tile = (old + 1) % tpb == 0;
+            const bool last_tile = old == before_last;
             if (last_tile) __hip_atomic_store(&P.h_done[rs0 + sl], bb + 1, __ATOMIC_RELAXED, __HIP_MEMORY_SCOPE_SYSTEM);
             if (stamp) {
                 st_stamp(&stamp[3], __builtin_amdgcn_s_memrealtime());
@@ -210,14 +251,16 @@
         };
         auto advance = [&] {
             j += rb;
-            uint32_t db = qb;
-            if (j >= tpb) {
-                j -= tpb;
-                db++;
-            }
-            b += db;
-            slot += db % n_slots;
-            if (slot >= n_slots) slot -= n_slots;
+            const bool carry = j >= tpb;
+            if (carry) j -= tpb;
+            b += carry ? qb + 1 : qb;
+            xs += carry ? ds1 : ds0;
+            lap += carry ? dl1 : dl0;
+            if (xs >= n_slots) {
+                xs -= n_slots;
+                lap++;
+            }
+            slot = slot0 + xs >= n_slots ? slot0 + xs - n_slots : slot0 + xs;
         };
         for (;;) {
             if (stamp && tid == 0) st_stamp(&stamp[0], __builtin_amdgcn_s_memrealtime());
@@ -229,8 +272,8 @@
                     s_door[2] = hp == 0 ? 1u : 0u;
                 }
                 lds_barrier();
-                posted = ((unsigned long long)s_door[1] << 32) | s_door[0];
-                const uint32_t leave = s_door[2];
+                posted = ((unsigned long long)lds_uni(&s_door[1]) << 32) | lds_uni(&s_door[0]);
+                const uint32_t leave = lds_uni(&s_door[2]);
                 lds_barrier();
                 if (leave) break;
             }
@@ -243,11 +286,11 @@
                 if (tid == 0)
                     s_door[3] = __hip_atomic_load(&P.h_n[rs0 + slot], __ATOMIC_RELAXED, __HIP_MEMORY_SCOPE_SYSTEM);
                 lds_barrier();
-                n = min(s_door[3], rg.n);
+                n = min(lds_uni(&s_door[3]), rg.n);
                 lds_barrier();
             }
             const uint32_t ntiles = (n + TILE - 1) / TILE;
-            const bool wrapped = b >= P.seq0r[r] + n_slots;
+            const bool wrapped = lap != 0;
             const bool sysld = P.sys_acquire == 3u || (P.sys_acquire == 4u && wrapped);
             if (P.sys_acquire == 1u || (P.sys_acquire == 2u && wrapped)) __builtin_amdgcn_fence(__ATOMIC_ACQUIRE, "");
             int tid_i = tid;
@@ -256,11 +299,29 @@
             const int wave_i = __builtin_amdgcn_readfirstlane(tid_i >> 6);
             bool ok = true;
             if constexpr (STEPS) {
-                if (j < ntiles) {
-                    const CopKBatch bt = pmd_batch(p, rg, slot, n, ntiles);
+                const bool tile_full = (j + 1) * TILE <= n, tile_some = j < ntiles;
+                const CopKBatch bt = pmd_batch(p, rg, slot, n, ntiles);
+                const uint32_t j_t = j;
+                if (COPK_PMD_UNI && COPK_PMD_PARK) {
+                    asm volatile("" : "+v"(b), "+v"(lap), "+v"(posted), "+v"(xs), "+v"(slot), "+v"(j));
+                    asm volatile("" : "+v"(qb), "+v"(rb), "+v"(ds0), "+v"(dl0), "+v"(ds1), "+v"(dl1), "+v"(slot0));
+                }
+                if (tile_some) {
                     constexpr int WIN = LPM == COPK_TBL_DIR ? COPK_PMD_WIN_DIR : COPK_PMD_WIN;
-                    if (sysld) tile_steps<FW, LPM, PPT, COPK_PMD_WT != 0, 1, WIN, LAY>(p, lc, bt, j, tid_i, lane_i, wave_i);
-                    else tile_steps<FW, LPM, PPT, COPK_PMD_WT != 0, 0, WIN, LAY>(p, lc, bt, j, tid_i, lane_i, wave_i);
+                    constexpr bool WT = COPK_PMD_WT != 0;
+                    if (tile_full) {
+                        if (sysld) tile_steps<FW, LPM, PPT, WT, 1, WIN, LAY, true>(p, lc, bt, j_t, tid_i, lane_i, wave_i);
+                        else tile_steps<FW, LPM, PPT, WT, 0, WIN, LAY, true>(p, lc, bt, j_t, tid_i, lane_i, wave_i);
+                    } else {
+                        if (sysld) tile_steps<FW, LPM, PPT, WT, 1, WIN, LAY>(p, lc, bt, j_t, tid_i, lane_i, wave_i);
+                        else tile_steps<FW, LPM, PPT, WT, 0, WIN, LAY>(p, lc, bt, j_t, tid_i, lane_i, wave_i);
+                    }
+                }
+                if (COPK_PMD_UNI && COPK_PMD_PARK) {
+                    b = uni64(b), lap = uni64(lap), posted = uni64(posted);
+                    xs = uni(xs), slot = uni(slot), j = uni(j);
+                    qb = uni(qb), rb = uni(rb), ds0 = uni(ds0), dl0 = uni(dl0), ds1 = uni(ds1), dl1 = uni(dl1);
+                    slot0 = uni(slot0);
                 }
             } else {
                 if (P.test_skip && r == 0 && b == 0 && j + 1 == P.test_skip) {
@@ -291,25 +352,24 @@
             advance();
         }
     };
-    constexpr bool DYN_OK = (PPT <= 2 || (COPK_PMD_WIN < PPT ? COPK_PMD_WIN : PPT) <= 2) && LAY == COPK_LAY_COALESCED;
     auto serve_dyn = [&](auto steps_c) {
-        constexpr bool STEPS = decltype(steps_c)::value && DYN_OK;
+        constexpr bool STEPS = decltype(steps_c)::value && dyn_ok<LAY, PPT>();
         if constexpr (STEPS) {
             constexpr int W = COPK_PMD_WIN < PPT ? COPK_PMD_WIN : PPT;
             const bool det = P.dyn == 2u;
-            const uint32_t nx = (!det && P.tk_lanes > 1 && tpb % P.tk_lanes == 0) ? P.tk_lanes : 1u;
+            const uint32_t nx = P.tk_nx;
             const uint32_t xl = wr % nx;
-            const uint32_t per = tpb / nx;
+            const uint32_t per = P.div_per.d;
             unsigned long long *ticket = P.d_ticket + ((size_t)r * COPK_PMD_TK_LANES + xl) * 16;
             uint32_t *s_tk = lc.s_misc + 72;
             unsigned long long *stamp = P.stamps ? P.stamps + (size_t)blockIdx.x * 8 : nullptr;
             const bool leader = wr % P.relay_stride == 0;
             unsigned long long posted = 0;
-            unsigned long long pend_old = 0, pend_b = 0;
+            unsigned long long pend_old = 0, pend_b = 0, pend_last = 0;
             uint32_t pend_sl = 0;
             bool pend = false;
             auto pend_flush = [&] {
-                if (pend && (pend_old + 1) % tpb == 0)
+                if (pend && pend_old == pend_last)
                     __hip_atomic_store(&P.h_done[rs0 + pend_sl], pend_b + 1, __ATOMIC_RELAXED,
                                        __HIP_MEMORY_SCOPE_SYSTEM);
                 pend = false;
@@ -317,7 +377,10 @@
             auto claim = [&](unsigned long long cur) {
                 return det ? cur + G : __hip_atomic_fetch_add(ticket, 1ull, __ATOMIC_RELAXED, __HIP_MEMORY_SCOPE_AGENT);
             };
-            auto tk_get = [&] { return ((unsigned long long)s_tk[1] << 32) | s_tk[0]; };
+            auto tk_get = [&] {
+                return ((unsigned long long)__builtin_amdgcn_readfirstlane(s_tk[1]) << 32) |
+                       __builtin_amdgcn_readfirstlane(s_tk[0]);
+            };
             if (tid == 0) {
                 const unsigned long long t0 = det ? (unsigned long long)wr : claim(0);
                 s_tk[0] = (uint32_t)t0;
@@ -330,14 +393,39 @@
             bool loaded = false;
             uint32_t n = rg.n, ntiles = (rg.n + TILE - 1) / TILE;
             const unsigned long long seq0 = P.seq0r[r];
+            const uint32_t slot0 = (uint32_t)(seq0 % n_slots);
+            struct Where {
+                unsigned long long b, lap;
+                uint32_t j, slot;
+            };
+            auto where = [&](unsigned long long t) {
+                Where w;
+                if ((t >> 32) == 0) {
+                    const uint32_t t32 = (uint32_t)t;
+                    const uint32_t x = copk_div(t32, P.div_per);
+                    const uint32_t lp = copk_div(x, P.div_slots);
+                    const uint32_t xs = x - lp * n_slots;
+                    w.b = seq0 + x;
+                    w.lap = lp;
+                    w.j = (t32 - x * per) * nx + xl;
+                    w.slot = slot0 + xs >= n_slots ? slot0 + xs - n_slots : slot0 + xs;
+                } else {
+                    const unsigned long long x = t / per;
+                    w.b = seq0 + x;
+                    w.lap = x / n_slots;
+                    w.j = (uint32_t)(t % per) * nx + xl;
+                    w.slot = (uint32_t)(w.b % n_slots);
+                }
+                return w;
+            };
             auto one = [&](u32x4 (&cur)[W][3], u32x4 (&nxt)[W][3]) -> bool {
                 int tid_i = tid;
                 asm volatile("" : "+v"(tid_i));
                 const int lane_i = tid_i & 63;
                 const int wave_i = __builtin_amdgcn_readfirstlane(tid_i >> 6);
-                const unsigned long long b = seq0 + T / per;
-                const uint32_t j = (uint32_t)(T % per) * nx + xl;
-                const uint32_t slot = (uint32_t)(b % n_slots);
+                const Where wt = where(T);
+                const unsigned long long b = wt.b;
+                const uint32_t j = wt.j, slot = wt.slot;
                 if (stamp && tid == 0) {
                     st_stamp(&stamp[0], __builtin_amdgcn_s_memrealtime());
                     st_stamp(&stamp[4], b);
@@ -352,8 +440,8 @@
                             s_door[2] = hp == 0 ? 1u : 0u;
                         }
                         lds_barrier();
-                        posted = ((unsigned long long)s_door[1] << 32) | s_door[0];
-                        const uint32_t leave = s_door[2];
+                        posted = ((unsigned long long)lds_uni(&s_door[1]) << 32) | lds_uni(&s_door[0]);
+                        const uint32_t leave = lds_uni(&s_door[2]);
                         lds_barrier();
                         if (leave) return true;
                     }
@@ -362,16 +450,19 @@
                         if (tid == 0)
                             s_door[3] = __hip_atomic_load(&P.h_n[rs0 + slot], __ATOMIC_RELAXED, __HIP_MEMORY_SCOPE_SYSTEM);
                         lds_barrier();
-                        n = min(s_door[3], rg.n);
+                        n = min(lds_uni(&s_door[3]), rg.n);
                         lds_barrier();
                     }
                     ntiles = (n + TILE - 1) / TILE;
-                    const bool wrapped = b >= seq0 + n_slots;
+                    const bool wrapped = wt.lap != 0;
                     if (P.sys_acquire == 1u || (P.sys_acquire == 2u && wrapped))
                         __builtin_amdgcn_fence(__ATOMIC_ACQUIRE, "");
                     const bool sysld = P.sys_acquire == 3u || (P.sys_acquire == 4u && wrapped);
                     step_prio<0>();
-                    if (j < ntiles)
+                    if ((j + 1) * TILE <= n)
+                        steps_load<PPT, 0, W, 2, COPK_PMD_WIN, true>(pmd_batch(p, rg, slot, n, ntiles), j, lane_i, wave_i,
+                                                                     cur, sysld);
+                    else if (j < ntiles)
                         steps_load<PPT, 0, W>(pmd_batch(p, rg, slot, n, ntiles), j, lane_i, wave_i, cur, sysld);
                 }
                 if (stamp && tid == 0) st_stamp(&stamp[1], __builtin_amdgcn_s_memrealtime());
@@ -382,22 +473,30 @@
                 }
                 lds_barrier();
                 const unsigned long long Tn = tk_get();
-                const unsigned long long bn = seq0 + Tn / per;
-                const uint32_t jn = (uint32_t)(Tn % per) * nx + xl;
-                const uint32_t sn = (uint32_t)(bn % n_slots);
+                const Where wn = where(Tn);
+                const unsigned long long bn = wn.b;
+                const uint32_t jn = wn.j, sn = wn.slot;
                 const bool pf = bn < posted && !P.h_n;
                 if (pf) {
-                    const bool wrapped = bn >= seq0 + n_slots;
+                    const bool wrapped = wn.lap != 0;
                     if (P.sys_acquire == 1u || (P.sys_acquire == 2u && wrapped))
                         __builtin_amdgcn_fence(__ATOMIC_ACQUIRE, "");
                     const bool sysld = P.sys_acquire == 3u || (P.sys_acquire == 4u && wrapped);
-                    if (jn < ntiles)
+                    if ((jn + 1) * TILE <= rg.n)
+                        steps_load<PPT, 0, W, 2, COPK_PMD_WIN, true>(pmd_batch(p, rg, sn, rg.n, ntiles), jn, lane_i,
+                                                                     wave_i, nxt, sysld);
+                    else if (jn < ntiles)
                         steps_load<PPT, 0, W>(pmd_batch(p, rg, sn, rg.n, ntiles), jn, lane_i, wave_i, nxt, sysld);
                 }
-                if (j < ntiles) {
-                    const bool sys_t = P.sys_acquire == 3u || (P.sys_acquire == 4u && b >= seq0 + n_slots);
-                    tile_steps_v<FW, LPM, PPT, COPK_PMD_WT != 0>(p, lc, pmd_batch(p, rg, slot, n, ntiles), j, tid_i,
-                                                                  lane_i, wave_i, cur, sys_t);
+                {
+                    constexpr bool WT = COPK_PMD_WT != 0;
+                    const bool sys_t = P.sys_acquire == 3u || (P.sys_acquire == 4u && wt.lap != 0);
+                    const CopKBatch bt = pmd_batch(p, rg, slot, n, ntiles);
+                    if ((j + 1) * TILE <= n)
+                        tile_steps_v<FW, LPM, PPT, WT, 2, COPK_PMD_WIN, COPK_PMD_STAGE_LIST, COPK_LAY_COALESCED, true>(
+                            p, lc, bt, j, tid_i, lane_i, wave_i, cur, sys_t);
+                    else if (j < ntiles)
+                        tile_steps_v<FW, LPM, PPT, WT>(p, lc, bt, j, tid_i, lane_i, wave_i, cur, sys_t);
                 }
                 if (stamp && tid == 0) st_stamp(&stamp[2], __builtin_amdgcn_s_memrealtime());
                 asm volatile("" ::: "memory");
@@ -407,6 +506,7 @@
                 if (tid == 0) {
                     pend_flush();
                     pend_old = atomicAdd(&P.slot_tiles[(size_t)(rs0 + slot) * P.slot_stride], 1ull);
+                    pend_last = (wt.lap + 1) * tpb - 1;
                     pend_b = b;
                     pend_sl = slot;
                     pend = true;
@@ -422,25 +522,29 @@
             }
         }
     };
-    if (steps_ok<FW, LPM, LAY, EXT>() && p.seg && p.compact && p.rec_paired && P.stepwise) {
-        if (DYN_OK && P.dyn) serve_dyn(std::integral_constant<bool, steps_ok<FW, LPM, LAY, EXT>()>{});
-        else serve(std::integral_constant<bool, steps_ok<FW, LPM, LAY, EXT>()>{});
-    } else {
-        serve(std::integral_constant<bool, false>{});
-    }
+    if constexpr (LOOP == LOOP_DYN) serve_dyn(std::integral_constant<bool, true>{});
+    else serve(std::integral_constant<bool, LOOP == LOOP_STEPS>{});
+}
+
+template <typename K>
+hipError_t pmd_kernel(K kern, const CopKPmd *p, uint32_t lds, hipStream_t s, int *occ)
+{
+    if (occ) return hipOccupancyMaxActiveBlocksPerMultiprocessor(occ, kern, BLOCK, lds);
+    hipLaunchKernelGGL(kern, dim3(p->n_work), dim3(BLOCK), lds, s, *p);
+    return hipGetLastError();
 }
 
 template <int FW, int LPM, int LAY, int PPT>
 hipError_t pmd_one(const CopKPmd *p, int ext, uint32_t lds, hipStream_t s, int *occ)
 {
-    if (occ) {
-        if (ext) return hipOccupancyMaxActiveBlocksPerMultiprocessor(occ, cop_pmd<FW, LPM, LAY, PPT, true>, BLOCK, lds);
-        return hipOccupancyMaxActiveBlocksPerMultiprocessor(occ, cop_pmd<FW, LPM, LAY, PPT, false>, BLOCK, lds);
+    if (ext) return pmd_kernel(cop_pmd<FW, LPM, LAY, PPT, true, LOOP_BODY>, p, lds, s, occ);
+    const int loop = pmd_loop_of<FW, LPM, LAY, PPT>(p, ext);
+    if constexpr (steps_ok<FW, LPM, LAY, false>()) {
+        if constexpr (dyn_ok<LAY, PPT>())
+            if (loop == LOOP_DYN) return pmd_kernel(cop_pmd<FW, LPM, LAY, PPT, false, LOOP_DYN>, p, lds, s, occ);
+        if (loop == LOOP_STEPS) return pmd_kernel(cop_pmd<FW, LPM, LAY, PPT, false, LOOP_STEPS>, p, lds, s, occ);
     }
-    const dim3 grid(p->n_work);
-    if (ext) hipLaunchKernelGGL((cop_pmd<FW, LPM, LAY, PPT, true>), grid, dim3(BLOCK), lds, s, *p);
-    else hipLaunchKernelGGL((cop_pmd<FW, LPM, LAY, PPT, false>), grid, dim3(BLOCK), lds, s, *p);
-    return hipGetLastError();
+    return pmd_kernel(cop_pmd<FW, LPM, LAY, PPT, false, LOOP_BODY>, p, lds, s, occ);
 }
 
 template <int FW, int LPM, int LAY>
@@ -514,10 +618,10 @@
     return pmd_dispatch(p, fw_mode, lpm_mode, layout, ppt, ext, lds_bytes, stream, nullptr);
 }
 
-extern "C" hipError_t copk_pmd_occupancy(int fw_mode, int lpm_mode, int layout, int ppt, int ext, uint32_t lds_bytes,
-                                         int *per_cu)
+extern "C" hipError_t copk_pmd_occupancy(const CopKPmd *p, int fw_mode, int lpm_mode, int layout, int ppt, int ext,
+                                         uint32_t lds_bytes, int *per_cu)
 {
     *per_cu = 0;
-    return pmd_dispatch(nullptr, fw_mode, lpm_mode, layout, ppt, ext, lds_bytes, nullptr, per_cu);
-}
-#endif
+    return pmd_dispatch(p, fw_mode, lpm_mode, layout, ppt, ext, lds_bytes, nullptr, per_cu);
+}
+#endif
diff --git a/ghost-dataplane_amd/csrc/cop_runtime.cpp b/ghost-dataplane_amd/csrc/cop_runtime.cpp
--- a/ghost-dataplane_amd/csrc/cop_runtime.cpp
+++ b/ghost-dataplane_amd/csrc/cop_runtime.cpp
@@ -2112,16 +2112,24 @@
     return rc ? rc : rrc;
 }
 
+static void pmd_loop(cop_pmd *m)
+{
+    m->P.stepwise = getenv("COP_PMD_STEPWISE") && !atoi(getenv("COP_PMD_STEPWISE")) ? 0u : 1u;
+    m->P.dyn = m->dyn ? 1u : m->pf ? 2u : 0u;
+}
+
 static void pmd_size(cop_pmd *m)
 {
     m->P.n_work = (uint32_t)m->c->ncu * m->per_cu;
     m->P.relay_stride = 257;
     if (const char *e = getenv("COP_PMD_RELAY_STRIDE")) m->P.relay_stride = std::max(1u, (uint32_t)atoi(e));
     m->P.poll_backoff = 3;
-    m->P.stepwise = getenv("COP_PMD_STEPWISE") && !atoi(getenv("COP_PMD_STEPWISE")) ? 0u : 1u;
-    m->P.dyn = m->dyn ? 1u : m->pf ? 2u : 0u;
+    pmd_loop(m);
     m->P.tk_lanes = COPK_PMD_TK_LANES;
     if (const char *e = getenv("COP_PMD_TK_LANES")) m->P.tk_lanes = atoi(e) == 1 ? 1u : (uint32_t)COPK_PMD_TK_LANES;
+    m->P.tk_nx = copk_pmd_tk_nx(m->P.dyn, m->P.tk_lanes, m->tpb);
+    m->P.div_per = copk_div_make(m->tpb / m->P.tk_nx);
+    m->P.div_slots = copk_div_make(m->n_slots);
     if (const char *e = getenv("COP_PMD_BACKOFF")) m->P.poll_backoff = std::min(64u, (uint32_t)atoi(e));
     m->P.sys_acquire = m->acquire;
     if (m->acquire == 4u) {
@@ -2379,9 +2387,12 @@
         }
         m->ext = (p.demux || p.port_stats || p.rule_hits || p.dbg) ? 1 : 0;
         int occ = 0;
-        hipError_t e = copk_pmd_occupancy(m->fw_mode, m->lpm_mode, m->layout, ppt, m->ext, m->lds_bytes, &occ);
+        pmd_loop(m);
+        hipError_t e = copk_pmd_occupancy(&m->P, m->fw_mode, m->lpm_mode, m->layout, ppt, m->ext, m->lds_bytes, &occ);
         if (e != hipSuccess || occ < 1) PMD_FAIL(set_err(c, -EIO, "pmd occupancy: %s (%d)", hipGetErrorString(e), occ));
         occ = std::min(occ, 6);
+        if (ppt == 4) occ = std::min(occ, 5);
+        if (ppt == 8) occ = std::min(occ, 4);
         if (p.dbg) occ = std::min(occ, 4);
         if (m->bins) occ = std::min(occ, 4);
         if (m->dyn) occ = std::min(occ, 5);
diff --git a/ghost-dataplane_amd/csrc/cop_tile.h b/ghost-dataplane_amd/csrc/cop_tile.h
--- a/ghost-dataplane_amd/csrc/cop_tile.h
+++ b/ghost-dataplane_amd/csrc/cop_tile.h
@@ -224,7 +224,37 @@
     else return (uint32_t)(k * BLOCK + wave * 64);
 }
 
-template <int PPT, int K0, int K1, int SYS = 2, int WIN = COPK_PMD_WIN>
+struct TileLoads {
+    StepOff f;
+    const uint8_t *p0;
+    __amdgpu_buffer_rsrc_t rs;
+    uint32_t s0;
+    uint32_t stride;
+};
+
+template <int PPT, int SYS>
+__device__ __forceinline__ TileLoads tile_loads(const CopKBatch &B, const StepGeom &sg, uint32_t base, int wave,
+                                                bool sys)
+{
+    TileLoads t;
+    t.f = step_voff(sg, B.stride);
+    t.stride = B.stride;
+    const uint32_t pb = base + step_off<PPT>(0, wave);
+    t.p0 = B.pkts + B.data_off + (size_t)pb * B.stride;
+    t.s0 = pb * B.stride;
+    if (SYS != 0 && sys) t.rs = sys_rsrc(B.pkts + B.data_off);
+    return t;
+}
+
+template <int PPT>
+__device__ __forceinline__ void load_step_k(const TileLoads &t, int k, int wave, bool sys, u32x4 (&v)[3])
+{
+    const uint32_t d = (step_off<PPT>(k, wave) - step_off<PPT>(0, wave)) * t.stride;
+    if (sys) load_step_full_sys(t.rs, t.s0 + d, t.f, v);
+    else load_step_full(t.p0 + d, t.f, v);
+}
+
+template <int PPT, int K0, int K1, int SYS = 2, int WIN = COPK_PMD_WIN, bool FULL = false>
 __device__ __forceinline__ void steps_load(const CopKBatch &B, uint32_t j, int lane, int wave,
                                            u32x4 (&v)[win_of<PPT, WIN>()][3], bool sys_rt = false)
 {
@@ -232,14 +262,20 @@
     static_assert(K1 <= win_of<PPT, WIN>(), "steps beyond the window");
     const StepGeom sg = step_geom(lane);
     const uint32_t base = j * (BLOCK * PPT);
-    const uint32_t last = B.n ? B.n - 1 : 0u;
-#pragma unroll
-    for (int k = K0; k < K1; k++)
-        load_step(sg, B.pkts + B.data_off, B.stride, base + step_off<PPT>(k, wave), last, v[k], sys);
+    if constexpr (FULL) {
+        const TileLoads tl = tile_loads<PPT, SYS>(B, sg, base, wave, sys);
+#pragma unroll
+        for (int k = K0; k < K1; k++) load_step_k<PPT>(tl, k, wave, sys, v[k]);
+    } else {
+        const uint32_t last = B.n ? B.n - 1 : 0u;
+#pragma unroll
+        for (int k = K0; k < K1; k++)
+            load_step(sg, B.pkts + B.data_off, B.stride, base + step_off<PPT>(k, wave), last, v[k], sys);
+    }
 }
 
 template <int FW, int LPM, int PPT, bool WT, int SYS = 2, int WIN = COPK_PMD_WIN,
-          bool STAGE_LIST = COPK_PMD_STAGE_LIST, int LAY = COPK_LAY_COALESCED>
+          bool STAGE_LIST = COPK_PMD_STAGE_LIST, int LAY = COPK_LAY_COALESCED, bool FULL = false>
 __device__ __forceinline__ void tile_steps_v(const CopKParams &p, const LdsCarve &lc, const CopKBatch &B, uint32_t j,
                                              int tid, int lane, int wave, u32x4 (&v)[win_of<PPT, WIN>()][3],
                                              bool sys_rt = false)
@@ -249,10 +285,31 @@
     const Tables &tb = lc.tb;
     constexpr int TILE = BLOCK * PPT;
     const uint32_t base = j * TILE;
-    const uint32_t last = B.n ? B.n - 1 : 0u;
+    const uint32_t last = FULL ? 0xFFFFFFFFu : B.n ? B.n - 1 : 0u;
     const StepGeom sg = step_geom(lane);
+    const StepSel ss = step_sel(sg);
+    TileLoads tl;
+    if constexpr (FULL && LAY != COPK_LAY_IMIX) tl = tile_loads<PPT, SYS>(B, sg, base, wave, sys);
+    auto load_k = [&](int k, u32x4 (&x)[3]) {
+        if constexpr (FULL && LAY != COPK_LAY_IMIX) load_step_k<PPT>(tl, k, wave, sys, x);
+        else load_step(sg, B.pkts + B.data_off, B.stride, base + step_off<PPT>(k, wave), last, x, sys);
+    };
+    auto valid_k = [&](int k) { return FULL || (base + step_off<PPT>(k, wave) + (uint32_t)lane < B.n && B.n != 0); };
     constexpr int W = win_of<PPT, WIN>();
-    Counts tot;
+    uint32_t n_in = 0, n_fwd = 0, n_dropfw = 0, n_parse = 0, n_noport = 0, n_notv4 = 0, n_rhit = 0;
+    auto counts_of = [&] {
+        Counts t;
+        t.rx = FULL ? (uint32_t)(PPT * 64) : n_in;
+        t.fwd = n_fwd;
+        t.dropfw = n_dropfw;
+        t.parse = n_parse;
+        t.noport = n_noport;
+        t.rhit = n_rhit;
+        t.total = FW != COPK_TBL_OFF ? t.rx - n_parse - n_noport : 0u;
+        t.notv4 = n_notv4;
+        return t;
+    };
+    constexpr bool SEGW = COPK_SEG_WAVE && PPT == WAVES;
     uint32_t *r = (uint32_t *)B.results;
     const int i2 = lane & 31;
     const bool staged = STAGE_LIST && B.fwd_idx && lc.cl.stage && !(COPK_XP & 4);
@@ -260,30 +317,30 @@
     auto flush = [&](int k, uint32_t len) {
         const uint32_t cc = (uint32_t)wave * 16u + (uint32_t)(lane & 15);
         const uint32_t pk = base + (uint32_t)k * BLOCK;
-        if (lane < 16 && cc * 4u < len)
-            st_list_chunk<WT>(&lc.cl.stage[k * BLOCK + cc * 4u], B.fwd_idx, pk + cc * 4u, B.n);
+        if (lane < 16 && cc * 4u < len) {
+            if (FULL) st_u32x4<WT>(*(const u32x4 *)&lc.cl.stage[k * BLOCK + cc * 4u], B.fwd_idx, (long)(pk + cc * 4u));
+            else st_list_chunk<WT>(&lc.cl.stage[k * BLOCK + cc * 4u], B.fwd_idx, pk + cc * 4u, B.n);
+        }
     };
     uint32_t run = 0;
     auto emit = [&](int k, bool valid0, uint32_t verdict0, uint32_t flags0, uint32_t port0, uint32_t rnh0) {
         const uint32_t pk0 = base + k * BLOCK;
         const uint32_t wb = base + step_off<PPT>(k, wave);
-        const bool valid[1] = {valid0};
-        const uint32_t verdict[1] = {verdict0}, flags[1] = {flags0};
-        const Counts c = wave_counts<FW, 1>(valid, verdict, flags);
-        tot.total += c.total;
-        tot.notv4 += c.notv4;
-        tot.fwd += c.fwd;
-        tot.dropfw += c.dropfw;
-        tot.parse += c.parse;
-        tot.noport += c.noport;
-        tot.rhit += c.rhit;
-        tot.rx += c.rx;
-        const unsigned long long bal = __ballot(valid0 && verdict0 == COPK_FORWARD);
-        if (lane == 0) {
-            lc.cl.cnt[k * WAVES + wave] = (uint32_t)__popcll(bal);
-            if (k == PPT - 1) {
-                const uint32_t c8[8] = {tot.total, tot.notv4, tot.fwd, tot.dropfw, tot.parse, tot.noport, tot.rhit,
-                                        tot.rx};
+        const unsigned long long in = FULL ? ~0ull : __ballot(valid0);
+        const unsigned long long bal = __ballot(verdict0 == COPK_FORWARD) & in;
+        if (!FULL) n_in += (uint32_t)__popcll(in);
+        n_fwd += (uint32_t)__popcll(bal);
+        n_dropfw += (uint32_t)__popcll(__ballot(verdict0 == COPK_DROP_FW) & in);
+        n_parse += (uint32_t)__popcll(__ballot(verdict0 == COPK_DROP_PARSE) & in);
+        n_noport += (uint32_t)__popcll(__ballot(verdict0 == COPK_DROP_NO_PORT) & in);
+        if (FW != COPK_TBL_OFF) n_notv4 += (uint32_t)__popcll(__ballot(verdict0 == COPK_DROP_NOT_IPV4) & in);
+        if (LPM != COPK_TBL_OFF) n_rhit += (uint32_t)__popcll(__ballot((flags0 & COPK_FLAG_ROUTE_HIT) != 0u) & in);
+        constexpr bool RED = !SEGW || !COPK_WAVE_COUNTERS || (COPK_XP & 4) != 0;
+        if ((!SEGW || RED) && lane == 0) {
+            if (!SEGW) lc.cl.cnt[k * WAVES + wave] = (uint32_t)__popcll(bal);
+            if (RED && k == PPT - 1) {
+                const Counts t = counts_of();
+                const uint32_t c8[8] = {t.total, t.notv4, t.fwd, t.dropfw, t.parse, t.noport, t.rhit, t.rx};
 #pragma unroll
                 for (int q = 0; q < 8; q++) lc.s_red[wave * 8 + q] = c8[q];
             }
@@ -293,7 +350,7 @@
         const uint32_t a2 = (uint32_t)__shfl((int)rx, 2 * i2 + 1), a3 = (uint32_t)__shfl((int)rnh0, 2 * i2 + 1);
         const uint32_t idx = wb + 2u * (uint32_t)i2;
         if (lane < 32 && !(COPK_XP & 2)) {
-            if (idx + 1 < B.n) st_u32x4<WT>(u32x4{a0, a1, a2, a3}, r, 2 * (long)idx);
+            if (FULL || idx + 1 < B.n) st_u32x4<WT>(u32x4{a0, a1, a2, a3}, r, 2 * (long)idx);
             else if (idx < B.n) st_u32x2<WT>(u32x2{a0, a1}, (u32x2 *)&r[2 * (size_t)idx]);
         }
         if (COPK_XP & 4) {
@@ -303,7 +360,7 @@
             }
             return;
         }
-        if constexpr (COPK_SEG_WAVE && PPT == WAVES) {
+        if constexpr (SEGW) {
             const uint32_t sb = base + (uint32_t)wave * COPK_SEG;
             const uint32_t rank = run + __builtin_amdgcn_mbcnt_hi((uint32_t)(bal >> 32),
                                                                   __builtin_amdgcn_mbcnt_lo((uint32_t)bal, 0u));
@@ -316,13 +373,18 @@
             if (k == PPT - 1) {
                 if (staged) {
                     asm volatile("" ::: "memory");
-                    if ((uint32_t)lane * 4u < run)
-                        st_list_chunk<WT>(&lc.cl.stage[wave * COPK_SEG + lane * 4], B.fwd_idx, sb + (uint32_t)lane * 4u,
-                                          B.n);
+                    if ((uint32_t)lane * 4u < run) {
+                        if (FULL)
+                            st_u32x4<WT>(*(const u32x4 *)&lc.cl.stage[wave * COPK_SEG + lane * 4], B.fwd_idx,
+                                         (long)(sb + (uint32_t)lane * 4u));
+                        else
+                            st_list_chunk<WT>(&lc.cl.stage[wave * COPK_SEG + lane * 4], B.fwd_idx,
+                                              sb + (uint32_t)lane * 4u, B.n);
+                    }
                 }
-                if (B.fwd_count && lane == 0 && sb < B.n) st_u32<WT>(run, B.fwd_count + sb / COPK_SEG);
+                if (B.fwd_count && lane == 0 && (FULL || sb < B.n)) st_u32<WT>(run, B.fwd_count + sb / COPK_SEG);
                 if (COPK_WAVE_COUNTERS) {
-                    counters_add_wave(p, tot, lane, blockIdx.x * WAVES + (uint32_t)wave);
+                    counters_add_wave(p, counts_of(), lane, blockIdx.x * WAVES + (uint32_t)wave);
                 } else {
                     lds_barrier();
                     counters_add(p, lc.s_red, tid);
@@ -347,7 +409,7 @@
         } else if (B.fwd_idx && ((bal >> lane) & 1ull)) {
             st_u32<WT>(pk0 + tid, &B.fwd_idx[pk0 + rank]);
         }
-        if (B.fwd_count && tid == 0 && pk0 < B.n) st_u32<WT>(all, B.fwd_count + pk0 / COPK_SEG);
+        if (B.fwd_count && tid == 0 && (FULL || pk0 < B.n)) st_u32<WT>(all, B.fwd_count + pk0 / COPK_SEG);
         if (k == PPT - 1) counters_add(p, lc.s_red, tid);
     };
     auto prio = [&](int k) {
@@ -377,11 +439,11 @@
             if (k < PPT) {
                 uint32_t w3[1], w6[1], w7[1], w8[1];
                 prio(k);
-                gather_step(sg, h, w3[0], w6[0], w7[0], w8[0]);
+                gather_step_sel(sg, ss, h, w3[0], w6[0], w7[0], w8[0]);
                 uint32_t verdict[1], port[1], fwe[1], lpe[1], lpe2[1], fwe2[1], src[1], dst[1];
                 pass1<FW, LPM, 1>(p, tb, w3, w6, w7, w8, verdict, port, src, dst, fwe, lpe, lpe2, fwe2);
                 a = St{w3[0], src[0], dst[0], verdict[0], port[0], fwe[0], lpe[0], lpe2[0],
-                       base + step_off<PPT>(k, wave) + (uint32_t)lane < B.n && B.n != 0, T8{false, 0ull}, BkQ{}};
+                       valid_k(k), T8{false, 0ull}, BkQ{}};
                 if (k + 1 < PPT) {
                     load_step_imix(sg, B.pkts, off, B.data_off, h, sys);
                     if (k + 2 < PPT) off = load_off_imix(B.offsets, base + step_off<PPT>(k + 2, wave), lane, last, sys);
@@ -410,10 +472,9 @@
         for (int k = 0; k < PPT; k++) {
             uint32_t w3[1], w6[1], w7[1], w8[1];
             prio(k);
-            gather_step(sg, v[k % W], w3[0], w6[0], w7[0], w8[0]);
-            if (k + W < PPT)
-                load_step(sg, B.pkts + B.data_off, B.stride, base + step_off<PPT>(k + W, wave), last, v[k % W], sys);
-            const bool valid[1] = {base + step_off<PPT>(k, wave) + (uint32_t)lane < B.n && B.n != 0};
+            gather_step_sel(sg, ss, v[k % W], w3[0], w6[0], w7[0], w8[0]);
+            if (k + W < PPT) load_k(k + W, v[k % W]);
+            const bool valid[1] = {valid_k(k)};
             uint32_t verdict[1], port[1], flags[1], rnh[1], fwe[1], lpe[1], lpe2[1], fwe2[1], src[1], dst[1], ct = 0,
                 cn = 0;
             if (COPK_XP & 1) {
@@ -441,14 +502,12 @@
             if (k < PPT) {
                 uint32_t w3[1], w6[1], w7[1], w8[1];
                 prio(k);
-                gather_step(sg, v[k % W], w3[0], w6[0], w7[0], w8[0]);
-                if (k + W < PPT)
-                    load_step(sg, B.pkts + B.data_off, B.stride, base + step_off<PPT>(k + W, wave), last, v[k % W],
-                              sys);
+                gather_step_sel(sg, ss, v[k % W], w3[0], w6[0], w7[0], w8[0]);
+                if (k + W < PPT) load_k(k + W, v[k % W]);
                 uint32_t verdict[1], port[1], fwe[1], lpe[1], lpe2[1], fwe2[1], src[1], dst[1];
                 pass1<FW, LPM, 1>(p, tb, w3, w6, w7, w8, verdict, port, src, dst, fwe, lpe, lpe2, fwe2);
                 a = St{w3[0], src[0], dst[0], verdict[0], port[0], fwe[0], lpe[0], lpe2[0],
-                       base + step_off<PPT>(k, wave) + (uint32_t)lane < B.n && B.n != 0, T8{false, 0ull}, BkQ{}};
+                       valid_k(k), T8{false, 0ull}, BkQ{}};
             }
             if (k >= 1 && k <= PPT) {
                 if constexpr (LPM == COPK_TBL_BKT) b.bq = bkt_pairs_issue(p.lpm_bpairs, b.lpe, b.verdict == COPK_FORWARD);
@@ -476,14 +535,15 @@
     step_prio<3>();
 }
 
-template <int FW, int LPM, int PPT, bool WT, int SYS, int WIN = COPK_PMD_WIN, int LAY = COPK_LAY_COALESCED>
+template <int FW, int LPM, int PPT, bool WT, int SYS, int WIN = COPK_PMD_WIN, int LAY = COPK_LAY_COALESCED,
+          bool FULL = false>
 __device__ __forceinline__ void tile_steps(const CopKParams &p, const LdsCarve &lc, const CopKBatch &B, uint32_t j,
                                            int tid, int lane, int wave)
 {
     u32x4 v[win_of<PPT, WIN>()][3];
     step_prio<0>();
-    if constexpr (LAY != COPK_LAY_IMIX) steps_load<PPT, 0, win_of<PPT, WIN>(), SYS, WIN>(B, j, lane, wave, v);
-    tile_steps_v<FW, LPM, PPT, WT, SYS, WIN, COPK_PMD_STAGE_LIST, LAY>(p, lc, B, j, tid, lane, wave, v);
+    if constexpr (LAY != COPK_LAY_IMIX) steps_load<PPT, 0, win_of<PPT, WIN>(), SYS, WIN, FULL>(B, j, lane, wave, v);
+    tile_steps_v<FW, LPM, PPT, WT, SYS, WIN, COPK_PMD_STAGE_LIST, LAY, FULL>(p, lc, B, j, tid, lane, wave, v);
 }
 
 template <int FW, int LPM, int LAY, int PPT, bool EXT, bool WT>
```

After: 65970. 1.8% lower.
